# levs57/halo2-liam-eagen-msm

Hardware: AMD Instinct MI355X
Metric: BN254 G1 MSM scalar-point-pairs/s (higher is better)
Workload: dtype u32 limbs (256-bit Montgomery integers)

## Files before the change

halo2_liam_eagen_msm_amd/csrc/kernels.cuh:

```cuda
#pragma once
#include "kernels_ec.cuh"
#include "inv29.cuh"

namespace lemsm {

__device__ __forceinline__ u32 extract_bits(const u32 (&s)[8], u32 bitpos, u32 c) {
  u32 li = bitpos >> 5, sh = bitpos & 31;
  u32 lo = 0, hi = 0;
#pragma unroll
  for (int i = 0; i < 8; i++) {
    lo = ((u32)i == li) ? s[i] : lo;
    hi = ((u32)i == li + 1) ? s[i] : hi;
  }
  u64 v = ((u64)hi << 32) | lo;
  return (u32)(v >> sh) & ((1u << c) - 1u);
}

struct KAdd { u32 k[8]; u32 order[8]; };

template <int MODE ,
          int BS = 256 >
__global__ __launch_bounds__(BS) void k_pip_digits(const uint4* __restrict__ scalars, KAdd kadd, GroupPlan pl,
                                                    uint16_t* __restrict__ dig16, unsigned long long* __restrict__ signbm,
                                                    u32* __restrict__ block_counts,
                                                    u32* __restrict__ bin_total, u32* __restrict__ err) {
  __shared__ u32 hist[MAX_BINS];
  const u32 tid = threadIdx.x, r = blockIdx.x;
  for (u32 i = tid; i < pl.nbins; i += BS) hist[i] = 0;
  __syncthreads();
  const u32 half = 1u << (pl.c - 1);
  u32 j0 = r * pl.spb, j1 = min(j0 + pl.spb, pl.n);
  for (u32 jb = j0 + tid; jb < j1; jb += BS * 4) {
    uint4 a[4], b[4];
#pragma unroll
    for (int u = 0; u < 4; u++) {
      u32 j = jb + (u32)BS * u;
      if (j < j1) { a[u] = scalars[2 * (size_t)j]; b[u] = scalars[2 * (size_t)j + 1]; }
      else { a[u] = make_uint4(0, 0, 0, 0); b[u] = a[u]; }
    }
#pragma unroll
    for (int u = 0; u < 4; u++) {
      u32 j = jb + (u32)BS * u;
      if (j >= j1) continue;
      u32 s[8] = {a[u].x, a[u].y, a[u].z, a[u].w, b[u].x, b[u].y, b[u].z, b[u].w};
      u32 bw = 0;
#pragma unroll
      for (int i = 0; i < 8; i++) { u32 dmy = __builtin_subc(s[i], kadd.order[i], bw, &bw); (void)dmy; }
      if (!bw) {
        atomicAdd(&err[0], 1u); atomicMax(&err[1], ~j);
#pragma unroll
        for (int i = 0; i < 8; i++) s[i] = 0;
      }
      u32 cy = 0;
#pragma unroll
      for (int i = 0; i < 8; i++) s[i] = __builtin_addc(s[i], kadd.k[i], cy, &cy);
      if (MODE == 2) {
#pragma unroll
        for (int w = 0; w < 15; w++) {
          if ((u32)w < pl.w0 || (u32)w >= pl.w1) continue;
          u32 raw = extract_bits(s, 17u * w, 17u);
          u32 sign = ((u32)w + 1 < pl.W && raw < 65536u) ? 1u : 0u;
          u32 mag = ((u32)w + 1 < pl.W) ? (sign ? 65536u - raw : raw - 65536u) : raw;
          dig16[(size_t)((u32)w - pl.w0) * pl.dstride + j] = (uint16_t)(sign ? mag - 1u : mag);
          unsigned long long bal = __ballot(sign != 0);
          if ((threadIdx.x & 63u) == 0) signbm[(size_t)((u32)w - pl.w0) * ((pl.n + 63) / 64) + (j >> 6)] = bal;
          if (mag) atomicAdd(&hist[((u32)w - pl.w0) * pl.BW + ((mag - 1u) >> pl.LB)], 1u);
        }
      } else if (MODE == 1) {
#pragma unroll
        for (int w = 0; w < 16; w++) {
          if ((u32)w < pl.w0 || (u32)w >= pl.w1) continue;
          u32 raw = (w & 1) ? (s[w >> 1] >> 16) : (s[w >> 1] & 0xffffu);
          dig16[(size_t)((u32)w - pl.w0) * pl.dstride + j] = (uint16_t)raw;
          u32 bucket = ((u32)w + 1 < pl.W) ? (raw < half ? half - raw : raw - half) : raw;
          if (bucket) atomicAdd(&hist[((u32)w - pl.w0) * pl.BW + ((bucket - 1u) >> pl.LB)], 1u);
        }
      } else {
        for (u32 w = pl.w0; w < pl.w1; w++) {
          u32 raw = extract_bits(s, w * pl.c, pl.c);
          dig16[(size_t)(w - pl.w0) * pl.dstride + j] = (uint16_t)raw;
          u32 bucket = (w + 1 < pl.W) ? (raw < half ? half - raw : raw - half) : raw;
          if (bucket) atomicAdd(&hist[(w - pl.w0) * pl.BW + ((bucket - 1u) >> pl.LB)], 1u);
        }
      }
    }
  }
  __syncthreads();
  for (u32 i = tid; i < pl.nbins; i += BS) {
    u32 cnt = hist[i];
    u32 wl = i / pl.BW, bin = i - wl * pl.BW;
    const size_t slot = ((size_t)wl * pl.nblk1 + r) * pl.BW + bin;
    block_counts[slot] = cnt;
    block_counts[(size_t)pl.nblk1 * pl.nbins + slot] = cnt ? atomicAdd(&bin_total[i], cnt) : 0u;
  }
}

struct PipDec {
  static constexpr bool VEC = true;
  const uint16_t* dig16;
  const unsigned long long* signbm;
  __device__ __forceinline__ void get(u32 j, u32 w, const GroupPlan& pl, u32& bucket, u32& sign) const {
    u32 raw = dig16[(size_t)(w - pl.w0) * pl.dstride + j];
    if (signbm) {
      sign = (u32)(signbm[(size_t)(w - pl.w0) * ((pl.n + 63) / 64) + (j >> 6)] >> (j & 63u)) & 1u;
      bucket = sign ? raw + 1u : raw;
      return;
    }
    const u32 half = 1u << (pl.c - 1);
    if (w + 1 < pl.W) {
      sign = raw < half ? 1u : 0u;
      bucket = sign ? half - raw : raw - half;
    } else { sign = 0; bucket = raw; }
  }
};
struct NegDec {
  static constexpr bool VEC = false;
  const uint8_t* digitsT;
  __device__ __forceinline__ void get(u32 j, u32 w, const GroupPlan& pl, u32& bucket, u32& sign) const {
    bucket = digitsT[(size_t)w * pl.nstride + j]; sign = 0;
  }
};

__device__ __forceinline__ u32 block_excl_scan_256(u32 v, u32* total, u32* wsum ) {
  const u32 lane = threadIdx.x & 63, wave = threadIdx.x >> 6;
  u32 x = v;
#pragma unroll
  for (int o = 1; o < 64; o <<= 1) {
    u32 y = __shfl_up(x, o);
    if (lane >= (u32)o) x += y;
  }
  if (lane == 63) wsum[wave] = x;
  __syncthreads();
  u32 base = 0, tot = 0;
#pragma unroll
  for (u32 w = 0; w < 4; w++) {
    u32 s = wsum[w];
    if (w < wave) base += s;
    tot += s;
  }
  __syncthreads();
  *total = tot;
  return base + x - v;
}

static const u32 BW_MAX = 512;
static const u32 STAGE = 4096;
static const u32 STAGE2 = 8192;

template <class Dec>
__global__ __launch_bounds__(256) void k_count1(Dec dec, GroupPlan pl, u32* __restrict__ block_counts,
                                                u32* __restrict__ bin_total) {
  __shared__ u32 hist[256];
  const u32 tid = threadIdx.x, wl = blockIdx.x, r = blockIdx.y, w = pl.w0 + wl;
  hist[tid] = 0;
  __syncthreads();
  u32 j0 = r * pl.spb, j1 = min(j0 + pl.spb, pl.n);
  constexpr int PER = STAGE / 256;
  u32 bk[PER];
#pragma unroll
  for (int k = 0; k < PER; k++) {
    u32 j = j0 + tid + 256u * k, sign;
    bk[k] = 0;
    if (j < j1) dec.get(j, w, pl, bk[k], sign);
  }
  const bool few = pl.BW <= 16u;
  const u32 rep = few ? (tid & 15u) << 4 : 0u;
#pragma unroll
  for (int k = 0; k < PER; k++)
    if (bk[k]) atomicAdd(&hist[rep + ((bk[k] - 1u) >> pl.LB)], 1u);
  __syncthreads();
  if (few) {
    u32 c = 0;
    if (tid < 16u) {
#pragma unroll
      for (int r = 0; r < 16; r++) c += hist[r * 16 + tid];
    }
    __syncthreads();
    if (tid < 16u) hist[tid] = c;
    __syncthreads();
  }
  if (tid < pl.BW) {
    u32 cnt = hist[tid];
    const size_t slot = ((size_t)wl * pl.nblk1 + r) * pl.BW + tid;
    block_counts[slot] = cnt;
    block_counts[(size_t)pl.nblk1 * pl.nbins + slot] = cnt ? atomicAdd(&bin_total[wl * pl.BW + tid], cnt) : 0u;
  }
}

__device__ __forceinline__ u32 block_excl_scan_1024(u32 v, u32* total, u32* wsum ) {
  const u32 lane = threadIdx.x & 63, wave = threadIdx.x >> 6;
  u32 x = v;
#pragma unroll
  for (int o = 1; o < 64; o <<= 1) {
    u32 y = __shfl_up(x, o);
    if (lane >= (u32)o) x += y;
  }
  if (lane == 63) wsum[wave] = x;
  __syncthreads();
  u32 base = 0, tot = 0;
  for (u32 w = 0; w < 16; w++) {
    u32 s = wsum[w];
    if (w < wave) base += s;
    tot += s;
  }
  __syncthreads();
  *total = tot;
  return base + x - v;
}

__global__ __launch_bounds__(1024) void k_binscan(GroupPlan pl, const u32* __restrict__ bin_total,
                                                  u32* __restrict__ bin_start, u32* __restrict__ tile_prefix,
                                                  u32* __restrict__ meta) {
  __shared__ u32 wsum[16];
  const u32 t = threadIdx.x;
  constexpr int PB = MAX_BINS / 1024;
  u32 cnt[PB], tl[PB], s = 0, st = 0;
#pragma unroll
  for (int k = 0; k < PB; k++) {
    u32 b = t * PB + k;
    cnt[k] = b < pl.nbins ? bin_total[b] : 0;
    tl[k] = (pl.bin_cap && cnt[k] <= pl.bin_cap) ? 0u : (cnt[k] + pl.T2 - 1) / pl.T2;
    s += cnt[k]; st += tl[k];
  }
  u32 tot, tott;
  u32 off = block_excl_scan_1024(s, &tot, wsum);
  u32 offt = block_excl_scan_1024(st, &tott, wsum);
#pragma unroll
  for (int k = 0; k < PB; k++) {
    u32 b = t * PB + k;
    if (b < pl.nbins) { bin_start[b] = off; tile_prefix[b] = offt; }
    off += cnt[k]; offt += tl[k];
  }
  if (t == 0) {
    bin_start[pl.nbins] = tot; tile_prefix[pl.nbins] = tott;
    meta[META_M] = tot; meta[META_TILES] = tott;
  }
}

template <class Dec, int STG , int BS = 256,
          bool LEAN = false >
__global__ __launch_bounds__(BS) void k_scatter1(Dec dec, GroupPlan pl, const u32* __restrict__ block_counts,
                                                 const u32* __restrict__ bin_start,
                                                 u32* __restrict__ entries, u32 xcd_windows ) {
  static_assert(BS == 256 || BS == 1024, "block size");
  static_assert(STG <= 16384, "jl field is 14 bits");
  static_assert(!LEAN || BS == 256, "the lean form is the 256-thread one");
  __shared__ __align__(8) u32 delta[BW_MAX];
  __shared__ __align__(8) u32 lcur[BW_MAX];
  __shared__ u32 wsum[16];
  __shared__ u32 stage[STG];
  const u32 tid = threadIdx.x;
  u32 wl, r;
  if (xcd_windows) {
    const u32 wpx = (pl.w1 - pl.w0 + 7u) >> 3, slot = blockIdx.x >> 3;
    wl = (blockIdx.x & 7u) + 8u * (slot % wpx); r = slot / wpx;
    if (wl >= pl.w1 - pl.w0) return;
  } else { wl = blockIdx.x; r = blockIdx.y; }
  const u32 w = pl.w0 + wl;
  const u32 lmask = (1u << pl.LB) - 1u;
  u32 j0 = r * pl.spb, j1 = min(j0 + pl.spb, pl.n);
  constexpr int PER = STG / BS;
  u32 bk[PER];
  u32 jl0, jls;
  if constexpr (Dec::VEC) {
    static_assert(PER == 16 || PER == 32, "digits per thread");
    jl0 = tid * PER; jls = 1;
    const u32 jb = j0 + jl0;
    uint4 dv[PER / 8];
    u32 sbits = 0;
    if (jb < j1) {
      const uint4* p = (const uint4*)(dec.dig16 + (size_t)wl * pl.dstride + jb);
#pragma unroll
      for (int v = 0; v < PER / 8; v++) dv[v] = p[v];
      if (dec.signbm) {
        const unsigned long long* sw = dec.signbm + (size_t)wl * ((pl.n + 63) / 64);
        if (PER == 16) sbits = ((const uint16_t*)sw)[jb >> 4]; else sbits = ((const u32*)sw)[jb >> 5];
      }
    } else {
#pragma unroll
      for (int v = 0; v < PER / 8; v++) dv[v] = make_uint4(0, 0, 0, 0);
    }
    const u32 half = 1u << (pl.c - 1);
    const bool top = !(w + 1 < pl.W);
#pragma unroll
    for (int k = 0; k < PER; k++) {
      const uint4 q4 = dv[k / 8];
      const u32 word = ((k / 2) % 4 == 0) ? q4.x : ((k / 2) % 4 == 1) ? q4.y : ((k / 2) % 4 == 2) ? q4.z : q4.w;
      const u32 raw = (k & 1) ? (word >> 16) : (word & 0xffffu);
      u32 bucket, sign;
      if (dec.signbm) { sign = (sbits >> k) & 1u; bucket = raw + sign; }
      else if (top) { sign = 0; bucket = raw; }
      else { sign = raw < half ? 1u : 0u; bucket = sign ? half - raw : raw - half; }
      bk[k] = (jb + (u32)k < j1 && bucket) ? (bucket | (sign << 31)) : 0u;
    }
  } else {
    jl0 = tid; jls = BS;
#pragma unroll
    for (int k = 0; k < PER; k++) {
      u32 j = j0 + tid + (u32)BS * k, b = 0, sgn = 0;
      if (j < j1) dec.get(j, w, pl, b, sgn);
      bk[k] = b ? (b | (sgn << 31)) : 0u;
    }
  }
  const size_t crow = ((size_t)wl * pl.nblk1 + r) * pl.BW;
  const u32* __restrict__ block_offs = block_counts + (size_t)pl.nblk1 * pl.nbins;
  u32 total;
  const bool few = !Dec::VEC && BS == 256 && !LEAN && pl.BW <= 16u;
  if (few) {
    lcur[tid] = 0;
    __syncthreads();
#pragma unroll
    for (int k = 0; k < PER; k++)
      if (bk[k]) atomicAdd(&lcur[((((bk[k] & 0x7fffffffu) - 1u) >> pl.LB) << 4) | (tid & 15u)], 1u);
    __syncthreads();
    const u32 v = lcur[tid];
    const u32 off = block_excl_scan_256(v, &total, wsum);
    lcur[tid] = off;
    const u32 b = tid >> 4;
    if ((tid & 15u) == 0 && b < pl.BW) delta[b] = bin_start[wl * pl.BW + b] + block_offs[crow + b] - off;
  } else
  if constexpr (LEAN) {
    const u32 b0 = 2u * tid;
    const bool h = b0 < pl.BW;
    const uint2 z2 = make_uint2(0u, 0u);
    const uint2 cnt = h ? *reinterpret_cast<const uint2*>(block_counts + crow + b0) : z2;
    const uint2 clm = h ? *reinterpret_cast<const uint2*>(block_offs + crow + b0) : z2;
    const uint2 bs = h ? *reinterpret_cast<const uint2*>(bin_start + (size_t)wl * pl.BW + b0) : z2;
    const u32 off0 = block_excl_scan_256(cnt.x + cnt.y, &total, wsum), off1 = off0 + cnt.x;
    *reinterpret_cast<uint2*>(&delta[b0]) = make_uint2(bs.x + clm.x - off0, bs.y + clm.y - off1);
    *reinterpret_cast<uint2*>(&lcur[b0]) = make_uint2(off0, off1);
  } else if constexpr (BS == 256) {
    const bool h0 = tid < pl.BW, h1 = tid + 256u < pl.BW;
    u32 cnt0 = h0 ? block_counts[crow + tid] : 0u, cnt1 = h1 ? block_counts[crow + tid + 256u] : 0u;
    u32 g0 = h0 ? bin_start[wl * pl.BW + tid] + block_offs[crow + tid] : 0u;
    u32 g1 = h1 ? bin_start[wl * pl.BW + tid + 256u] + block_offs[crow + tid + 256u] : 0u;
    u32 total0, total1;
    u32 off0 = block_excl_scan_256(cnt0, &total0, wsum);
    u32 off1 = block_excl_scan_256(cnt1, &total1, wsum) + total0;
    total = total0 + total1;
    delta[tid] = g0 - off0; delta[tid + 256u] = g1 - off1;
    lcur[tid] = off0; lcur[tid + 256u] = off1;
  } else {
    const bool h0 = tid < pl.BW;
    u32 cnt0 = h0 ? block_counts[crow + tid] : 0u;
    u32 g0 = h0 ? bin_start[wl * pl.BW + tid] + block_offs[crow + tid] : 0u;
    u32 off0 = block_excl_scan_1024(cnt0, &total, wsum);
    if (tid < BW_MAX) { delta[tid] = g0 - off0; lcur[tid] = off0; }
  }
  __syncthreads();
#pragma unroll
  for (int k = 0; k < PER; k++) {
    if (bk[k]) {
      u32 kk = (bk[k] & 0x7fffffffu) - 1u, b = kk >> pl.LB;
      u32 q = atomicAdd(&lcur[few ? ((b << 4) | (tid & 15u)) : b], 1u);
      if constexpr (LEAN) stage[q] = (bk[k] & 0x80000000u) | (jl0 + jls * (u32)k) | (b << 14) | ((kk & lmask) << 24);
      else stage[q] = (jl0 + jls * (u32)k) | ((kk & lmask) << 14) | ((bk[k] >> 31) << 21) | (b << 22);
    }
  }
  __syncthreads();
  if constexpr (LEAN) {
    u32 v[PER];
#pragma unroll
    for (int k = 0; k < PER; k++) { const u32 q = tid + (u32)BS * k; v[k] = q < total ? stage[q] : 0u; }
#pragma unroll
    for (int k = 0; k < PER; k++) {
      const u32 q = tid + (u32)BS * k;
      if (q < total) entries[delta[(v[k] >> 14) & 511u] + q] = (v[k] & 0xff003fffu) + j0;
    }
  } else {
    for (u32 q = tid; q < total; q += BS) {
      u32 v = stage[q];
      entries[delta[v >> 22] + q] = (j0 + (v & 0x3fffu)) | (((v >> 14) & 127u) << 24) | (((v >> 21) & 1u) << 31);
    }
  }
}

__global__ __launch_bounds__(256) void k_tilemap(GroupPlan pl, const u32* __restrict__ bin_start,
                                                 const u32* __restrict__ tile_prefix, const u32* __restrict__ meta,
                                                 uint4* __restrict__ tile_info) {
  u32 t = blockIdx.x * 256 + threadIdx.x;
  if (t >= pl.max_tiles) return;
  if (t >= meta[META_TILES]) { tile_info[t] = make_uint4(0, 0, 0, 0); return; }
  u32 lo = 0, hi = pl.nbins;
  while (hi - lo > 1) {
    u32 mid = (lo + hi) >> 1;
    if (tile_prefix[mid] <= t) lo = mid; else hi = mid;
  }
  u32 off = bin_start[lo] + (t - tile_prefix[lo]) * pl.T2;
  u32 end = min(off + pl.T2, bin_start[lo + 1]);
  tile_info[t] = make_uint4(lo, off, end, 1u);
}
__device__ __forceinline__ bool locate_tile(const uint4* __restrict__ tile_info, u32 t, u32& bin, u32& off, u32& end) {
  uint4 ti = tile_info[t];
  bin = ti.x; off = ti.y; end = ti.z;
  return ti.w != 0;
}

__global__ __launch_bounds__(256) void k_count2(GroupPlan pl, const u32* __restrict__ entries,
                                                const uint4* __restrict__ tile_info, u32* __restrict__ bucket_count) {
  __shared__ u32 hist[1u << MAX_LB];
  const u32 tid = threadIdx.x;
  for (u32 t = blockIdx.x; t < pl.max_tiles; t += gridDim.x) {
    u32 bin, off, end;
    if (!locate_tile(tile_info, t, bin, off, end)) return;
    if (tid < (1u << MAX_LB)) hist[tid] = 0;
    __syncthreads();
    constexpr int PER = STAGE2 / 256;
    u32 e[PER];
#pragma unroll
    for (int k = 0; k < PER; k++) { u32 i = off + tid + 256u * k; e[k] = i < end ? entries[i] : 0xffffffffu; }
#pragma unroll
    for (int k = 0; k < PER; k++) { u32 i = off + tid + 256u * k; if (i < end) atomicAdd(&hist[(e[k] >> 24) & 127u], 1u); }
    __syncthreads();
    if (tid < (1u << pl.LB)) {
      u32 cnt = hist[tid];
      if (cnt) atomicAdd(&bucket_count[(bin << pl.LB) + tid], cnt);
    }
    __syncthreads();
  }
}

__global__ __launch_bounds__(256) void k_bucketscan(GroupPlan pl, const u32* __restrict__ bin_start,
                                                    const u32* __restrict__ bucket_count,
                                                    u32* __restrict__ bucket_start) {
  __shared__ u32 ex[256];
  __shared__ u32 wsum[4];
  const u32 tid = threadIdx.x;
  const u32 key = blockIdx.x * 256 + tid;
  const u32 nkeys = pl.nbins << pl.LB;
  u32 cnt = key < nkeys ? bucket_count[key] : 0u;
  u32 total;
  u32 e = block_excl_scan_256(cnt, &total, wsum);
  ex[tid] = e;
  __syncthreads();
  if (key < nkeys) {
    u32 first = tid & ~((1u << pl.LB) - 1u);
    const u32 b0 = bin_start[key >> pl.LB];
    if (!(pl.bin_cap && bin_start[(key >> pl.LB) + 1] - b0 <= pl.bin_cap))
      bucket_start[key] = b0 + (e - ex[first]);
  }
  if (key == 0) bucket_start[nkeys] = bin_start[pl.nbins];
}

__global__ __launch_bounds__(256) void k_scatter2(GroupPlan pl, const u32* __restrict__ entries,
                                                  const uint4* __restrict__ tile_info, const u32* __restrict__ bucket_start,
                                                  u32* __restrict__ bucket_cursor, u32* __restrict__ sorted) {
  __shared__ u32 hist[256];
  __shared__ u32 lstart[257];
  __shared__ u32 delta[256];
  __shared__ u32 wsum[4];
  __shared__ u32 stage[STAGE2];
  const u32 tid = threadIdx.x;
  for (u32 t = blockIdx.x; t < pl.max_tiles; t += gridDim.x) {
    u32 bin, off, end;
    if (!locate_tile(tile_info, t, bin, off, end)) return;
    hist[tid] = 0;
    __syncthreads();
    constexpr int PER = STAGE2 / 256;
    u32 e[PER], rk[PER];
#pragma unroll
    for (int k = 0; k < PER; k++) { u32 i = off + tid + 256u * k; e[k] = i < end ? entries[i] : 0xffffffffu; }
#pragma unroll
    for (int k = 0; k < PER; k++) {
      u32 i = off + tid + 256u * k;
      rk[k] = i < end ? atomicAdd(&hist[(e[k] >> 24) & 127u], 1u) : 0u;
    }
    __syncthreads();
    u32 cnt = tid < (1u << pl.LB) ? hist[tid] : 0u;
    u32 total;
    u32 o = block_excl_scan_256(cnt, &total, wsum);
    lstart[tid] = o;
    if (tid == 255) lstart[256] = total;
    u32 key = (bin << pl.LB) + tid;
    delta[tid] = cnt ? bucket_start[key] + atomicAdd(&bucket_cursor[key], cnt) - o : 0u;
    __syncthreads();
#pragma unroll
    for (int k = 0; k < PER; k++) {
      u32 i = off + tid + 256u * k;
      if (i < end) {
        u32 l = (e[k] >> 24) & 127u;
        stage[lstart[l] + rk[k]] = e[k];
      }
    }
    __syncthreads();
    for (u32 q = tid; q < total; q += 256) {
      u32 v = stage[q];
      sorted[delta[(v >> 24) & 127u] + q] = v & 0x80ffffffu;
    }
    __syncthreads();
  }
}

static const u32 BIN_CAP = 36864;
static const u32 BIN_CAP_SMALL = 8192;
template <u32 CAP>
__global__ __launch_bounds__(1024) void k_binsort(GroupPlan pl, const u32* __restrict__ entries, const u32* __restrict__ bin_start,
                                                  u32* __restrict__ sorted, u32* __restrict__ bucket_start) {
  __shared__ u32 stage[CAP];
  __shared__ u32 hist[256];
  __shared__ u32 lstart[256];
  __shared__ u32 wsum[4];
  const u32 tid = threadIdx.x, bin = blockIdx.x;
  const u32 off = bin_start[bin], end = bin_start[bin + 1], cnt = end - off;
  if (cnt > pl.bin_cap) return;
  const u32 nl = 1u << pl.LB, lmask = nl - 1u;
  if (tid < 256) hist[tid] = 0;
  __syncthreads();
  constexpr int PER = CAP / 1024;
  u32 e[PER], rk[PER];
#pragma unroll
  for (int k = 0; k < PER; k++) { u32 i = off + tid + 1024u * k; e[k] = i < end ? entries[i] : 0u; }
#pragma unroll
  for (int k = 0; k < PER; k++) {
    u32 i = off + tid + 1024u * k;
    rk[k] = i < end ? atomicAdd(&hist[(e[k] >> 24) & lmask], 1u) : 0u;
  }
  __syncthreads();
  if (tid < 256) {
    u32 c = tid < nl ? hist[tid] : 0u, total;
    const u32 lane = tid & 63, wave = tid >> 6;
    u32 x = c;
#pragma unroll
    for (int o = 1; o < 64; o <<= 1) { u32 y = __shfl_up(x, o); if (lane >= (u32)o) x += y; }
    if (lane == 63) wsum[wave] = x;
    lstart[tid] = x - c;
    (void)total;
  }
  __syncthreads();
  const u32 wb1 = wsum[0], wb2 = wb1 + wsum[1], wb3 = wb2 + wsum[2];
  if (tid < nl) {
    u32 l = tid, base = l < 64 ? 0u : (l < 128 ? wb1 : (l < 192 ? wb2 : wb3));
    bucket_start[(bin << pl.LB) + l] = off + base + lstart[l];
  }
#pragma unroll
  for (int k = 0; k < PER; k++) {
    u32 i = off + tid + 1024u * k;
    if (i < end) {
      u32 l = (e[k] >> 24) & lmask, base = l < 64 ? 0u : (l < 128 ? wb1 : (l < 192 ? wb2 : wb3));
      stage[base + lstart[l] + rk[k]] = e[k] & 0x80ffffffu;
    }
  }
  __syncthreads();
  for (u32 q = tid; q < cnt; q += 1024) sorted[off + q] = stage[q];
}

__global__ void k_copy_points(const CopyTask* __restrict__ tasks, u32 ntasks, u32 nwin, u32 pt_bytes, char* __restrict__ arena) {
  u32 gid = blockIdx.x * blockDim.x + threadIdx.x;
  u32 wpp = pt_bytes / 16;
  u32 word = gid % wpp; u32 r = gid / wpp;
  u32 ti = r / nwin, w = r - ti * nwin;
  if (ti >= ntasks) return;
  CopyTask tk = tasks[ti];
  uint4 v = make_uint4(0, 0, 0, 0);
  if (tk.src_idx < tk.src_valid_idx)
    v = reinterpret_cast<const uint4*>(arena + ((size_t)tk.src_off + (size_t)w * tk.src_wstride + tk.src_idx) * pt_bytes)[word];
  reinterpret_cast<uint4*>(arena + ((size_t)tk.dst_off + (size_t)w * tk.dst_wstride) * pt_bytes)[word] = v;
}

__global__ __launch_bounds__(256) void k_negbase_digits(const uint4* __restrict__ scalars, u32 n, u32 base, u32 d,
                                                        const u32* __restrict__ bound , int check_range,
                                                        uint8_t* __restrict__ digits, uint8_t* __restrict__ digitsT,
                                                        u32* __restrict__ err, u32 row_begin, u32 row_end ,
                                                        const uint8_t* __restrict__ negative = nullptr ,
                                                        uint8_t* __restrict__ trunc = nullptr ) {
  u32 j = blockIdx.x * 256 + threadIdx.x;
  if (j >= n) return;
  uint4 a = scalars[2 * (size_t)j], b = scalars[2 * (size_t)j + 1];
  u32 s[8] = {a.x, a.y, a.z, a.w, b.x, b.y, b.z, b.w};
  u32 bw = 0;
#pragma unroll
  for (int i = 0; i < 8; i++) { u32 dummy = __builtin_subc(s[i], bound[i], bw, &bw); (void)dummy; }
  bool in_range = bw != 0;
  if (check_range && !in_range) { atomicMin(&err[0], j); }
  u32 h[16];
#pragma unroll
  for (int i = 0; i < 8; i++) { h[2 * i] = s[i] & 0xffffu; h[2 * i + 1] = s[i] >> 16; }
  bool neg = negative ? negative[j] != 0 : false;
  {
    u32 nz0 = 0;
#pragma unroll
    for (int k = 0; k < 16; k++) nz0 |= h[k];
    if (!nz0) neg = false;
  }
  const float rb = 1.0f / (float)base;
  const u32 shift = (base & (base - 1u)) == 0 ? (u32)__builtin_ctz(base) : 0u;
  u32 i_begin = 0;
  if (shift && !(s[4] | s[5] | s[6] | s[7])) {
    u32 m0 = s[0], m1 = s[1], m2 = s[2], m3 = s[3];
    for (u32 i = 0; i < d; i++) {
      const u32 rem = m0 & (base - 1u);
      m0 = __builtin_amdgcn_alignbit(m1, m0, shift); m1 = __builtin_amdgcn_alignbit(m2, m1, shift);
      m2 = __builtin_amdgcn_alignbit(m3, m2, shift); m3 >>= shift;
      u32 digit;
      if (!neg) { digit = rem; neg = true; }
      else {
        digit = rem ? base - rem : 0u;
        if (rem) {
          m0 += 1u; const u32 c0 = m0 == 0u; m1 += c0; const u32 c1 = c0 & (m1 == 0u); m2 += c1; const u32 c2 = c1 & (m2 == 0u); m3 += c2;
        }
        neg = false;
      }
      if (!(m0 | m1 | m2 | m3)) neg = false;
      if (digits) digits[(size_t)j * d + i] = (uint8_t)digit;
      if (digitsT && i >= row_begin && i < row_end) digitsT[(size_t)i * n + j] = (uint8_t)digit;
    }
    h[0] = m0 & 0xffffu; h[1] = m0 >> 16; h[2] = m1 & 0xffffu; h[3] = m1 >> 16; h[4] = m2 & 0xffffu; h[5] = m2 >> 16; h[6] = m3 & 0xffffu; h[7] = m3 >> 16;
    i_begin = d;
  }
  for (u32 i = i_begin; i < d; i++) {
    u32 rem = 0;
    if (shift) {
      rem = h[0] & (base - 1u);
#pragma unroll
      for (int k = 0; k < 16; k++) {
        u32 nxt = k < 15 ? h[k + 1] : 0u;
        h[k] = ((h[k] | (nxt << 16)) >> shift) & 0xffffu;
      }
    } else {
#pragma unroll
      for (int k = 15; k >= 0; k--) {
        u32 cur = (rem << 16) | h[k];
        u32 q = (u32)((float)cur * rb);
        int r = (int)cur - (int)(q * base);
        if (r < 0) { q--; r += (int)base; }
        if (r >= (int)base) { q++; r -= (int)base; }
        h[k] = q; rem = (u32)r;
      }
    }
    u32 digit;
    if (!neg) { digit = rem; neg = true; }
    else {
      digit = rem ? base - rem : 0u;
      if (rem) {
        u32 cy = 1;
#pragma unroll
        for (int k = 0; k < 16; k++) { u32 v = h[k] + cy; h[k] = v & 0xffffu; cy = v >> 16; }
      }
      neg = false;
    }
    u32 nz = 0;
#pragma unroll
    for (int k = 0; k < 16; k++) nz |= h[k];
    if (!nz) neg = false;
    if (digits) digits[(size_t)j * d + i] = (uint8_t)digit;
    if (digitsT && i >= row_begin && i < row_end) digitsT[(size_t)i * n + j] = (uint8_t)digit;
  }
  u32 nz = 0;
#pragma unroll
  for (int k = 0; k < 16; k++) nz |= h[k];
  if (nz) { atomicAdd(&err[1], 1u); atomicMin(&err[2], j); }
  if (trunc) trunc[j] = nz ? 1 : 0;
}

struct WitnessPow { unsigned long long lo; long long hi; u32 ovf; u32 pad; };

__device__ __forceinline__ bool add_i128(unsigned long long& lo, long long& hi, unsigned long long blo, long long bhi) {
  unsigned long long rlo = lo + blo;
  long long rhi = (long long)((unsigned long long)hi + (unsigned long long)bhi + (rlo < lo ? 1ull : 0ull));
  bool ovf = ((hi ^ rhi) & (bhi ^ rhi)) < 0;
  lo = rlo; hi = rhi;
  return ovf;
}

__global__ __launch_bounds__(256) void k_scalar_witness(const uint4* __restrict__ scalars, const uint8_t* __restrict__ negative,
                                                        const uint8_t* __restrict__ digits ,
                                                        const uint8_t* __restrict__ trunc, u32 n, u32 base, u32 d, u32 logtable,
                                                        u32 num_limbs, const WitnessPow* __restrict__ powtab,
                                                        char* __restrict__ out, unsigned long long* __restrict__ fail) {
  const u32 j = blockIdx.x * 256 + threadIdx.x;
  if (j >= n) return;
  const u32 cols = num_limbs + 1;
  char* cells = out + (size_t)j * base * cols * 24;
  auto cell = [&](u32 r, u32 c) -> char* { return cells + ((size_t)r * cols + c) * 24; };
  for (u32 r = 0; r < base; r++)
    for (u32 c = 0; c < cols; c++) {
      u32* w = reinterpret_cast<u32*>(cell(r, c));
      w[0] = w[1] = w[2] = w[3] = w[4] = 0;
      w[5] = (c == 0) ? (r == 0 ? 0u : 1u) : 2u;
    }
  auto report = [&](u32 code) { atomicMin(fail, ((unsigned long long)j << 4) | code); };
  if (trunc[j]) { report(1); return; }
  auto add_value = [&](char* c, const WitnessPow& pw) -> bool {
    unsigned long long* v = reinterpret_cast<unsigned long long*>(c);
    unsigned long long lo = v[0]; long long hi = (long long)v[1];
    if (pw.ovf) return true;
    bool o = add_i128(lo, hi, pw.lo, pw.hi);
    v[0] = lo; v[1] = (unsigned long long)hi;
    return o;
  };
  auto add_mask = [&](char* c, u32 k) -> bool {
    if (k >= 32) return true;
    u32* m = reinterpret_cast<u32*>(c + 16);
    u32 a = *m, r = a + (1u << k);
    *m = r;
    return r < a;
  };
  for (u32 i = 0; i < d; i++) {
    u32 dig = digits[(size_t)j * d + i];
    if (!dig) continue;
    const u32 id = dig - 1, k = i % logtable;
    if (add_value(cell(id + 1, 0), powtab[i])) { report(3); return; }
    if (powtab[k].ovf) { report(3); return; }
    if (k + 1 > num_limbs) { report(2); return; }
    if (add_value(cell(id + 1, k + 1), powtab[k])) { report(3); return; }
    if (add_mask(cell(id + 1, k + 1), k)) { report(3); return; }
    if (add_value(cell(0, k + 1), powtab[k])) { report(3); return; }
    if (add_mask(cell(0, k + 1), k)) { report(3); return; }
  }
  {
    uint4 a = scalars[2 * (size_t)j];
    unsigned long long lo = ((unsigned long long)a.y << 32) | a.x, hi = ((unsigned long long)a.w << 32) | a.z;
    if (negative && negative[j]) { lo = ~lo + 1ull; hi = ~hi + (lo == 0 ? 1ull : 0ull); }
    unsigned long long* v = reinterpret_cast<unsigned long long*>(cell(0, 0));
    v[0] = lo; v[1] = hi;
  }
}

template <class F>
__global__ __launch_bounds__(256) void k_table_entries(u32 base, unsigned long long id0, u32 count, uint4* __restrict__ out) {
  const u32 t = blockIdx.x * 256 + threadIdx.x;
  if (t >= count) return;
  typedef typename F::fe fe;
  unsigned long long id = id0 + t;
  fe acc, one, b, bm;
  F::set_zero(acc); F::set_one(one);
  F::set_zero(bm);
  for (int bit = 7; bit >= 0; bit--) { F::add(bm, bm, bm); if ((base >> bit) & 1u) F::add(bm, bm, one); }
  F::neg(b, bm);
  int l = 64 - (id ? __clzll((long long)id) : 64);
  for (int i = l - 1; i >= 0; i--) {
    if ((id >> i) & 1ull) F::add(acc, acc, one);
    F::mul(acc, acc, b);
  }
  F::store(out + 2 * (size_t)t, acc);
}

template <class F, int KB>
__global__ __launch_bounds__(256) void k_jac_to_affine(const uint4* __restrict__ jac, u32 n,
                                                       uint4* __restrict__ aff, char* __restrict__ scratch) {
  typedef typename F::fe fe;
  const u32 t = blockIdx.x * 256 + threadIdx.x;
  const u32 nthreads = gridDim.x * 256;
  const u64 j0 = (u64)t * KB;
  if (j0 >= n) return;
  const u32 cnt = (u32)min((u64)KB, (u64)n - j0);
  fe acc; F::set_one(acc);
  for (u32 k = 0; k < cnt; k++) {
    fe z; F::load(z, jac + (j0 + k) * 6 + 4);
    F::store(scratch + ((size_t)k * nthreads + t) * 32, acc);
    if (!F::is_zero(z)) F::mul(acc, acc, z);
  }
  fe inv; inv_via_lazy<F>(inv, acc);
  for (u32 k = cnt; k-- > 0;) {
    fe x, y, z, pref;
    const uint4* p = jac + (j0 + k) * 6;
    F::load(z, p + 4);
    uint4* o = aff + (j0 + k) * 4;
    if (F::is_zero(z)) {
      o[0] = make_uint4(0, 0, 0, 0); o[1] = o[0]; o[2] = o[0]; o[3] = o[0];
      continue;
    }
    F::load(x, p); F::load(y, p + 2);
    F::load(pref, scratch + ((size_t)k * nthreads + t) * 32);
    fe zi, zi2, zi3;
    F::mul(zi, inv, pref);
    F::mul(inv, inv, z);
    F::sqr(zi2, zi); F::mul(zi3, zi2, zi);
    F::mul(x, x, zi2); F::mul(y, y, zi3);
    F::store(o, x); F::store(o + 2, y);
  }
}

template <class F>
__global__ void k_dbg_montmul(const uint4* __restrict__ a, const uint4* __restrict__ b, uint4* __restrict__ out, u32 n) {
  u32 i = blockIdx.x * blockDim.x + threadIdx.x;
  if (i >= n) return;
  typename F::fe x, y, r;
  F::load(x, a + 2 * (size_t)i); F::load(y, b + 2 * (size_t)i);
  F::mul(r, x, y);
  F::store(out + 2 * (size_t)i, r);
}
template <class F>
__global__ void k_dbg_fieldop(int op, const uint4* __restrict__ a, const uint4* __restrict__ b, uint4* __restrict__ out, u32 n) {
  u32 i = blockIdx.x * blockDim.x + threadIdx.x;
  if (i >= n) return;
  typename F::fe x, y, r;
  F::load(x, a + 2 * (size_t)i); F::load(y, b + 2 * (size_t)i);
  if (op == 0) F::add(r, x, y);
  else if (op == 1) F::sub(r, x, y);
  else if (op == 2) F::neg(r, x);
  else if (op == 3) F::inv(r, x);
  else F::sqr(r, x);
  F::store(out + 2 * (size_t)i, r);
}
template <class F>
__global__ void k_dbg_pointop(int op, const char* __restrict__ acc_in, const char* __restrict__ q_in, char* __restrict__ out, u32 n) {
  typedef XYZZ<F> G;
  u32 i = blockIdx.x * blockDim.x + threadIdx.x;
  if (i >= n) return;
  typename G::pt acc; G::load(acc, acc_in + (size_t)i * 128);
  if (op == 0) {
    typename F::fe x, y; F::load(x, q_in + (size_t)i * 64); F::load(y, q_in + (size_t)i * 64 + 32);
    if (!(F::is_zero(x) && F::is_zero(y))) G::madd(acc, x, y);
  } else {
    typename G::pt q; G::load(q, q_in + (size_t)i * 128);
    G::add(acc, q);
  }
  G::store(out + (size_t)i * 128, acc);
}

}
```

halo2_liam_eagen_msm_amd/csrc/lemsm.hip:

```cpp
#include <hip/hip_runtime.h>
#include <math.h>
#include <stdio.h>
#include <stdlib.h>
#include <string.h>

#include <algorithm>
#include <cmath>
#include <map>
#include <string>
#include <vector>

#include "../../include/lemsm.h"
#include "hostmath.hpp"
#include "hostpool.hpp"
#include "hosttail.hpp"
#include <memory>
#include "kernels.cuh"
#include "rccl_dyn.hpp"
#include "roctx_dyn.hpp"
#include "divisor.cuh"
#include <rocprim/rocprim.hpp>
#include <chrono>
#include <functional>
#include <thread>

using namespace lemsm;

namespace {

typedef Field32<FqParams> FqDev;
typedef Field32<FrParams> FrDev;
typedef XYZZ<FqDev> GqStrict;
typedef XYZZ<FrDev> GrStrict;
typedef XYZZ29<Field29<Fq29Params>> GqLazy;
typedef XYZZ29<Field29<Fr29Params>> GrLazy;

const u32 ORDER_R[8] = {0xf0000001u, 0x43e1f593u, 0x79b97091u, 0x2833e848u, 0x8181585du, 0xb85045b6u, 0xe131a029u, 0x30644e72u};
const u32 ORDER_P[8] = {0xd87cfd47u, 0x3c208c16u, 0x6871ca8du, 0x97816a91u, 0x8181585du, 0xb85045b6u, 0xe131a029u, 0x30644e72u};
const u32 BOUND_R[8] = {0xc7b81b1bu, 0xc6fb4e9fu, 0xeeb859fcu, 0x6f4d8248u, 0, 0, 0, 0};
const u32 BOUND_P[8] = {0xc7b81b1cu, 0xc6fb4e9fu, 0xeeb859fcu, 0x6f4d8248u, 0, 0, 0, 0};

const u32* order_of(int curve) { return curve == LEMSM_BN254_G1 ? ORDER_R : ORDER_P; }
const u32* bound_of(int curve) { return curve == LEMSM_BN254_G1 ? BOUND_R : BOUND_P; }

}
#define LEMSM_EXTERN_G(G)                                                                                   \
  extern template __global__ void lemsm::k_merge_pairs<G>(GroupPlan, u32, MqLayout, const u32*, const u32*, const u32*, const char*, char*, u32*, uint4*); \
  extern template __global__ void lemsm::k_merge_serial<G>(u32, MqLayout, const u32*, const uint4*, const char*, char*); \
  extern template __global__ void lemsm::k_merge_waves<G>(u32, MqLayout, const u32*, const uint4*, const char*, char*, char*, u32*); \
  extern template __global__ void lemsm::k_merge_final<G>(u32, MqLayout, const u32*, const uint4*, const char*, char*, u32*); \
  extern template __global__ void lemsm::k_pyramid<G>(const PyrTask*, u32, u32, u32, char*, u32); \
  extern template __global__ void lemsm::k_pyramid_first2<G>(PyrFirst2Args, const u32*, char*, u32*); \
  extern template __global__ void lemsm::k_pyramid_tail<G>(const PyrTask*, PyrTailArgs, const CopyTaskPod*, u32, char*, u32);
#define LEMSM_EXTERN_ACC(G, W) \
  extern template __global__ void lemsm::k_accum1<G, W>(GroupPlan, const u32*, const u32*, u32*, const uint4*, char*, u32*, char*);
LEMSM_EXTERN_G(GqStrict) LEMSM_EXTERN_G(GrStrict) LEMSM_EXTERN_G(GqLazy) LEMSM_EXTERN_G(GrLazy)
LEMSM_EXTERN_ACC(GqStrict, 4) LEMSM_EXTERN_ACC(GrStrict, 4)
LEMSM_EXTERN_ACC(GqLazy, 2) LEMSM_EXTERN_ACC(GqLazy, 3) LEMSM_EXTERN_ACC(GqLazy, 4)
LEMSM_EXTERN_ACC(GrLazy, 2) LEMSM_EXTERN_ACC(GrLazy, 3) LEMSM_EXTERN_ACC(GrLazy, 4)
extern template __global__ void lemsm::k_accum1<GqLazy, 3, true>(GroupPlan, const u32*, const u32*, u32*, const uint4*, char*, u32*, char*);
extern template __global__ void lemsm::k_accum1<GrLazy, 3, true>(GroupPlan, const u32*, const u32*, u32*, const uint4*, char*, u32*, char*);
extern template __global__ void lemsm::k_accum1<GqLazy, 3, true, true>(GroupPlan, const u32*, const u32*, u32*, const uint4*, char*, u32*, char*);
extern template __global__ void lemsm::k_accum1<GrLazy, 3, true, true>(GroupPlan, const u32*, const u32*, u32*, const uint4*, char*, u32*, char*);
extern template __global__ void lemsm::k_convert_points<Field29<Fq29Params>>(const uint4*, uint4*, u32);
extern template __global__ void lemsm::k_convert_points<Field29<Fr29Params>>(const uint4*, uint4*, u32);
namespace {

struct DevBuf {
  void* p = nullptr;
  size_t cap = 0;
};


struct PyrCacheEntry { DevBuf buf; PyrPlan pp; };

}

struct HostStage { const uint8_t* h_scalars; const void* h_points; char* d_scalars; char* d_points; };

struct lemsm_ctx {
  int device = 0;
  u32 num_cus = 256;
  hipStream_t stream = nullptr;
  hipStream_t stream_sort = nullptr;
  hipStream_t stream_tail = nullptr;
  std::vector<hipEvent_t> evpool;
  hipEvent_t wait_accum = nullptr;
  hipEvent_t ev_call_done = nullptr;
  hipEvent_t ev_batch_up = nullptr;
  hipEvent_t dw_ev[2] = {nullptr, nullptr};
  hipEvent_t ev[5] = {nullptr, nullptr, nullptr, nullptr, nullptr};
  DevBuf ws;
  DevBuf in_s;
  DevBuf in_p;
  DevBuf in_aux;
  DevBuf gather;
  DevBuf fail_buf;
  DevBuf dw_tab, dw_arena, dw_tmp;
  u32 dw_logn = 0, dw_gexp = 0;
  double dw_ntt_ms = 0; u64 dw_ntt_bytes = 0, dw_ntt_bflies = 0; u32 dw_reuse_levels = 0;
  double dw_phase_ms[4] = {0, 0, 0, 0};
  ncclComm_t comm = nullptr; int comm_size = 1, comm_rank = 0;
  int plan_world = 1;
  u32* h_small = nullptr;
  lemsm_ctx* peer = nullptr;
  void* h_pin = nullptr; size_t h_pin_cap = 0;
  std::unique_ptr<lemsm::host::Pool> pool;
  std::string last_error;
  long opt_host_threads = 0;
  long opt_window_bits = 0, opt_chunk = 0, opt_tile = 0, opt_field = 0, opt_accum_waves = 0, opt_groups = 0, opt_host_slab_bits = 0, opt_slab_bits = 0, opt_abi_points = 0, opt_stage2x = 0, opt_xcd_windows = 0, opt_entry_ring = 0, opt_validate_points = 0, opt_pyr_fuse = 0, opt_ntt_tiled = 0, opt_ws_canary = 0, opt_binsort = 0, opt_dw_wrap = 0, opt_dw_fuse = 0, opt_dw_kb = 0, opt_merge_slice = 0, opt_merge_wave_th = 0, opt_dbg_repeat = 0, opt_pyr_first2 = 0, opt_dw_reuse = 0, opt_dw_pw_lazy = 0, opt_dw_halves = 0, opt_dw_ntt_lazy = 0, opt_slab_tail = 0, opt_pyr_quad = 0, opt_scatter_lean = 0;
  u32 plan_slab_n = 0;
  bool plan_ring = false;
  const struct HostStage* host_stage = nullptr;
  double t_total_ms = 0, t_accum_ms = 0; int n_accum = 0;
  double host_us[4] = {0, 0, 0, 0};
  uint32_t dbg_stamps[8] = {0, 0, 0, 0, 0, 0, 0, 0};
  uint64_t dbg_merge[4] = {0, 0, 0, 0};
  double accum_clock_mhz = 0;
  size_t bad_index = 0;
  size_t truncated = 0;
  std::map<std::vector<u32>, PyrCacheEntry> pyr_cache;
};

namespace {

#define HIPCHK(ctx, expr)                                                                   \
  do {                                                                                      \
    hipError_t e_ = (expr);                                                                 \
    if (e_ != hipSuccess) {                                                                 \
      (ctx)->last_error = std::string(#expr) + ": " + hipGetErrorString(e_);                \
      return LEMSM_ERR_HIP;                                                                 \
    }                                                                                       \
  } while (0)

int fail(lemsm_ctx* ctx, int code, const std::string& msg) {
  if (ctx) ctx->last_error = msg;
  return code;
}

int reserve(lemsm_ctx* ctx, DevBuf& b, size_t bytes) {
  if (b.cap >= bytes) return LEMSM_OK;
  if (b.p) { HIPCHK(ctx, hipFree(b.p)); b.p = nullptr; b.cap = 0; }
  size_t want = bytes + bytes / 8 + 4096;
  hipError_t e = hipMalloc(&b.p, want);
  if (e != hipSuccess) { b.p = nullptr; return fail(ctx, LEMSM_ERR_NOMEM, "hipMalloc failed: " + std::string(hipGetErrorString(e))); }
  b.cap = want;
  return LEMSM_OK;
}

int reserve_pinned(lemsm_ctx* ctx, size_t bytes) {
  if (ctx->h_pin_cap >= bytes) return LEMSM_OK;
  if (ctx->h_pin) { HIPCHK(ctx, hipHostFree(ctx->h_pin)); ctx->h_pin = nullptr; ctx->h_pin_cap = 0; }
  size_t want = bytes + bytes / 4 + 4096;
  hipError_t e = hipHostMalloc(&ctx->h_pin, want, hipHostMallocDefault);
  if (e != hipSuccess) { ctx->h_pin = nullptr; return fail(ctx, LEMSM_ERR_NOMEM, "hipHostMalloc failed: " + std::string(hipGetErrorString(e))); }
  ctx->h_pin_cap = want;
  return LEMSM_OK;
}

void host_parallel(lemsm_ctx* ctx, int njobs, const std::function<void(int)>& fn) {
  if (!ctx || njobs <= 1 || ctx->opt_host_threads == 1) { for (int i = 0; i < njobs; i++) fn(i); return; }
  int want = ctx->opt_host_threads > 1 ? (int)ctx->opt_host_threads : std::min(8, lemsm::host::Pool::usable_cpus());
  if (!ctx->pool || ctx->pool->workers() != want - 1) ctx->pool.reset(new lemsm::host::Pool(std::max(0, want - 1)));
  ctx->pool->run(njobs, fn);
}

bool geq8(const u32* a, const u32* b) {
  for (int i = 7; i >= 0; i--) { if (a[i] > b[i]) return true; if (a[i] < b[i]) return false; }
  return true;
}
void add8(u32* r, const u32* a, const u32* b) {
  u64 c = 0;
  for (int i = 0; i < 8; i++) { c += (u64)a[i] + b[i]; r[i] = (u32)c; c >>= 32; }
}
u32 logb_ceil8(const u32* x, u32 base) {
  u32 m[8]; memcpy(m, x, 32); u32 i = 0;
  for (;;) {
    u32 nz = 0; for (int k = 0; k < 8; k++) nz |= m[k];
    if (!nz) break;
    u64 rem = 0;
    for (int k = 7; k >= 0; k--) { u64 cur = (rem << 32) | m[k]; m[k] = (u32)(cur / base); rem = cur % base; }
    i++;
  }
  return i;
}
u32 next_pow2(u32 x) { u32 p = 1; while (p < x) p <<= 1; return p; }
u32 ilog2(u32 x) { u32 l = 0; while ((1u << l) < x) l++; return l; }

struct MsmPlan {
  u32 c, W, nb, nbp, L;
  u32 kadd[8];
};

u32 choose_c(const lemsm_ctx* ctx, size_t n) {
  if (ctx && ctx->opt_window_bits >= 2 && ctx->opt_window_bits <= 17) return (u32)ctx->opt_window_bits;
  u32 lg = 0; while (((size_t)1 << (lg + 1)) <= n) lg++;
  if (lg >= 24) return (ctx && ctx->plan_world > 1) ? 16u : 17u;
  int c = (int)lg - 3;
  if (c < 3) c = 3;
  if (c > 16) c = 16;
  return (u32)c;
}

u32 host_slab_log(const lemsm_ctx* ctx, size_t n) {
  u32 lg = 0; while (((size_t)2 << lg) <= n) lg++;
  u32 auto_log = std::min(21u, std::max(19u, lg >= 2 ? lg - 2 : 0u));
  if (ctx->host_stage && !ctx->host_stage->h_points) auto_log = std::min(22u, std::max(19u, lg >= 2 ? lg - 2 : 0u));
  return std::min<u32>(MAX_SLAB_LOG, ctx->opt_host_slab_bits ? (u32)ctx->opt_host_slab_bits : auto_log);
}

MsmPlan make_msm_plan(const lemsm_ctx* ctx, int curve, size_t n) {
  MsmPlan p; memset(&p, 0, sizeof p);
  size_t n_pass = n;
  if (ctx && ctx->host_stage) n_pass = std::min(n, (size_t)1 << host_slab_log(ctx, n));
  else if (ctx && ctx->opt_slab_bits) n_pass = std::min(n, (size_t)1 << ctx->opt_slab_bits);
  p.c = choose_c(ctx, n_pass);
  p.nb = 1u << (p.c - 1);
  p.nbp = p.nb; p.L = ilog2(p.nbp);
  const u32* order = order_of(curve);
  for (u32 W = (254 + p.c - 1) / p.c;; W++) {
    u32 K[8] = {0, 0, 0, 0, 0, 0, 0, 0};
    for (u32 w = 0; w + 1 < W; w++) {
      u32 bit = w * p.c + p.c - 1;
      if (bit < 256) K[bit >> 5] |= 1u << (bit & 31);
    }
    u32 s[9]; u64 cy = 0;
    for (int i = 0; i < 8; i++) { cy += (u64)order[i] + K[i]; s[i] = (u32)cy; cy >>= 32; }
    s[8] = (u32)cy;
    u32 sh = p.c * (W - 1);
    bool fits = true;
    if (s[8]) fits = false;
    u64 top = 0; bool big = false;
    for (int bit = 255; bit >= (int)sh; bit--) {
      u32 b = (s[bit >> 5] >> (bit & 31)) & 1u;
      if (top >> 62) big = true;
      top = (top << 1) | b;
    }
    if (big || top > p.nb) fits = false;
    if (sh >= 256) { fits = true; }
    if (fits) { p.W = W; memcpy(p.kadd, K, 32); break; }
  }
  if (p.c == 17 && p.W != 15) {
    lemsm_ctx tmp_opts; tmp_opts.opt_window_bits = 16;
    return make_msm_plan(&tmp_opts, curve, n);
  }
  return p;
}

template <class F> struct FieldTag {};

size_t align_up(size_t x, size_t a) { return (x + a - 1) / a * a; }

struct GroupWs {
  u32* err;
  char* arena;
  u32* bin_total; u32* bin_cursor; u32* bin_start; u32* tile_prefix; u32* meta;
  u32* bucket_count; u32* bucket_cursor; u32* bucket_start;
  u32* block_counts;
  uint16_t* dig16;
  unsigned long long* signbm;
  uint4* tile_info;
  u32* entries; u32* sorted;
  u32* rec_key; char* rec_pt;
  u32* mq_cnt; uint4* mq_items; char* mq_partial; MqLayout mq;
  size_t zero_begin, zero_bytes;
  size_t zero_bytes_counters;
  size_t total;
  std::vector<size_t> guards;
};

MqLayout make_mq_layout(const lemsm_ctx* ctx, u32 nthr1) {
  return make_mq_layout_t(nthr1, ctx && ctx->opt_merge_slice ? (u32)ctx->opt_merge_slice : 512u,
                          ctx && ctx->opt_merge_wave_th ? (u32)ctx->opt_merge_wave_th - 1u : 2048u);
}

const size_t WS_GUARD = 256;
GroupWs carve(char* base, const GroupPlan& pl, const ArenaLayout& ar, const MqLayout& mq, size_t ptb, bool guard = false) {
  GroupWs w; size_t off = 0;
  auto take = [&](size_t bytes) {
    size_t o = off;
    if (guard) { size_t g = align_up(off + bytes, 16); w.guards.push_back(g); off = align_up(g + WS_GUARD, 256); }
    else off = align_up(off + bytes, 256);
    return o;
  };
  u32 NBpad = pl.nbins << pl.LB;
  size_t z0 = off;
  size_t o_err = take(64);
  size_t o_mqcnt = take(MQ_WORDS * 4);
  size_t o_bin_total = take(MAX_BINS * 4), o_bin_cursor = take(MAX_BINS * 4);
  size_t o_bcount = take((size_t)NBpad * 4), o_bcursor = take((size_t)NBpad * 4);
  size_t o_arena = take((size_t)ar.total_points * ptb);
  size_t zend = o_arena + (size_t)(ar.apyr_off - ar.bucket_off) * ptb;
  w.zero_bytes_counters = o_arena - z0;
  size_t o_bin_start = take((MAX_BINS + 1) * 4), o_tile_prefix = take((MAX_BINS + 1) * 4), o_meta = take(64);
  size_t o_bstart = take(((size_t)NBpad + 1) * 4);
  size_t o_blockc = take((size_t)pl.nblk1 * pl.nbins * 8);
  size_t o_dig = take(pl.c ? (size_t)pl.dstride * (pl.w1 - pl.w0) * 2 + 64 : 16);
  size_t o_tinfo = take((size_t)pl.max_tiles * 16 + 16);
  size_t o_sbm = take(pl.c == 17 ? (size_t)(pl.w1 - pl.w0) * ((pl.n + 63) / 64) * 8 + 16 : 16);
  size_t Mmax = (size_t)pl.n * (pl.w1 - pl.w0);
  size_t o_entries = take(Mmax * 4 + 4 * (size_t)pl.L1 + 512), o_sorted = take(Mmax * 4 + 4 * (size_t)pl.L1 + 512);
  w.mq = mq;
  size_t o_rk = take((size_t)pl.nthr1 * 4 + 16), o_rp = take(2 * (size_t)pl.nthr1 * ptb + 256);
  size_t o_mqi = take(((size_t)mq.offF + mq.capF) * 16), o_mqp = take((size_t)mq.capP * ptb + 256);
  w.total = off;
  if (base) {
    w.err = (u32*)(base + o_err);
    w.bin_total = (u32*)(base + o_bin_total); w.bin_cursor = (u32*)(base + o_bin_cursor);
    w.bucket_count = (u32*)(base + o_bcount); w.bucket_cursor = (u32*)(base + o_bcursor);
    w.arena = base + o_arena;
    w.bin_start = (u32*)(base + o_bin_start); w.tile_prefix = (u32*)(base + o_tile_prefix); w.meta = (u32*)(base + o_meta);
    w.bucket_start = (u32*)(base + o_bstart); w.block_counts = (u32*)(base + o_blockc); w.dig16 = (uint16_t*)(base + o_dig); w.tile_info = (uint4*)(base + o_tinfo); w.signbm = (unsigned long long*)(base + o_sbm);
    w.entries = (u32*)(base + o_entries); w.sorted = (u32*)(base + o_sorted);
    w.rec_key = (u32*)(base + o_rk); w.rec_pt = base + o_rp;
    w.mq_cnt = (u32*)(base + o_mqcnt); w.mq_items = (uint4*)(base + o_mqi); w.mq_partial = base + o_mqp;
  }
  w.zero_begin = z0; w.zero_bytes = zend - z0;
  return w;
}

u32 choose_lb(const lemsm_ctx* ctx, u32 nb, u32 n, u32 d) {
  if (ctx && ctx->plan_slab_n) n = ctx->plan_slab_n;
  u32 LB = 0;
  while (((nb + (1u << LB) - 1) >> LB) > 256 && LB < MAX_LB) LB++;
  if (d == 0 && ctx && ctx->opt_binsort != 2 && LB > 0) {
    const u32 cap = ctx->opt_binsort > 2 ? std::min((u32)ctx->opt_binsort, (u32)BIN_CAP) : (u32)BIN_CAP;
    const u32 BW = (nb + (1u << LB) - 1) >> LB;
    if ((u64)n / BW > (u64)cap * 9 / 10 && 2 * BW <= BW_MAX && (u64)n / (2 * BW) <= (u64)cap * 9 / 10) LB--;
  }
  return LB;
}

GroupPlan make_group_plan(const lemsm_ctx* ctx, u32 n, u32 c, u32 nb, u32 W, u32 w0, u32 w1, u32 d) {
  GroupPlan g; memset(&g, 0, sizeof g);
  g.n = n; g.c = c; g.nb = nb; g.W = W; g.w0 = w0; g.w1 = w1; g.d = d; g.nstride = n;
  u32 LB = choose_lb(ctx, nb, n, d);
  g.LB = LB;
  g.BW = (nb + (1u << LB) - 1) >> LB;
  g.nbw = g.BW << LB;
  g.NB = (w1 - w0) * g.nbw;
  g.nbins = (w1 - w0) * g.BW;
  u32 spb = (n + 1023) / 1024;
  spb = std::max(256u, std::min((u32)STAGE, spb));
  spb = (spb + 255) / 256 * 256;
  if (n >= (1u << 16)) spb = STAGE;
  if (n >= (1u << 16) && d == 0 && ctx->opt_stage2x == 4) spb = 4 * STAGE;
  if (n >= (1u << 16) && d == 0 && ctx->opt_stage2x == 2) spb = 2 * STAGE;
  g.spb = spb;
  g.dstride = (n + 63u) / 64u * 64u;
  g.nblk1 = (n + spb - 1) / spb;
  if (g.nblk1 == 0) g.nblk1 = 1;
  size_t Mmax = (size_t)n * (w1 - w0);
  u32 T2 = ctx->opt_tile > 0 ? std::min((u32)ctx->opt_tile, (u32)STAGE2) : (u32)STAGE2;
  g.T2 = T2;
  g.max_tiles = (u32)(Mmax / T2) + g.nbins + 1;
  g.bin_cap = ctx->opt_binsort == 2 ? 0u : (ctx->opt_binsort > 2 ? std::min((u32)ctx->opt_binsort, (u32)BIN_CAP) : (u32)BIN_CAP);
  if (g.bin_cap == BIN_CAP && g.BW && (u64)n * 3 / 2 / g.BW <= BIN_CAP_SMALL) g.bin_cap = BIN_CAP_SMALL;
  u32 L1;
  if (ctx->opt_chunk > 0) L1 = (u32)ctx->opt_chunk;
  else {
    size_t target = (size_t)256 * 4 * 3 * 64 * 2;
    size_t l = (Mmax + target - 1) / target;
    L1 = (u32)std::max((size_t)8, std::min((size_t)256, l));
  }
  if (ctx->plan_ring && ctx->opt_chunk == 0 && L1 >= 128) L1 = (L1 + 15u) & ~15u;
  g.L1 = L1;
  g.nthr1 = (u32)((Mmax + L1 - 1) / L1);
  if (g.nthr1 == 0) g.nthr1 = 1;
  return g;
}

u32 max_group_windows(const lemsm_ctx* ctx, u32 nb, u32 n, u32 d) {
  u32 LB = choose_lb(ctx, nb, n, d);
  u32 BW = (nb + (1u << LB) - 1) >> LB;
  u32 cap = MAX_BINS / BW;
  return cap == 0 ? 1 : cap;
}

struct PipProvider {
  const uint4* scalars; KAdd kadd;
  typedef PipDec Dec;
  int prepare(lemsm_ctx*, hipStream_t st, const GroupPlan& pl, uint16_t* dig16, unsigned long long* signbm, u32* block_counts,
              u32* bin_total, u32* err, Dec& dec) const {
    dec.dig16 = dig16; dec.signbm = nullptr;
    if (pl.c == 17) {
      dec.signbm = signbm;
      if (pl.nblk1 < 2048)
        hipLaunchKernelGGL((k_pip_digits<2, 1024>), dim3(pl.nblk1), dim3(1024), 0, st, scalars, kadd, pl, dig16, signbm, block_counts, bin_total, err);
      else
        hipLaunchKernelGGL((k_pip_digits<2>), dim3(pl.nblk1), dim3(256), 0, st, scalars, kadd, pl, dig16, signbm, block_counts, bin_total, err);
    } else if (pl.c == 16 && pl.W == 16) {
      if (pl.nblk1 < 1024)
        hipLaunchKernelGGL((k_pip_digits<1, 1024>), dim3(pl.nblk1), dim3(1024), 0, st, scalars, kadd, pl, dig16, signbm, block_counts, bin_total, err);
      else
        hipLaunchKernelGGL((k_pip_digits<1>), dim3(pl.nblk1), dim3(256), 0, st, scalars, kadd, pl, dig16, signbm, block_counts, bin_total, err);
    } else {
      if (pl.nblk1 < 1024)
        hipLaunchKernelGGL((k_pip_digits<0, 1024>), dim3(pl.nblk1), dim3(1024), 0, st, scalars, kadd, pl, dig16, signbm, block_counts, bin_total, err);
      else
        hipLaunchKernelGGL((k_pip_digits<0>), dim3(pl.nblk1), dim3(256), 0, st, scalars, kadd, pl, dig16, signbm, block_counts, bin_total, err);
    }
    return LEMSM_OK;
  }
};
struct NegProvider {
  const uint8_t* digitsT;
  typedef NegDec Dec;
  int prepare(lemsm_ctx*, hipStream_t st, const GroupPlan& pl, uint16_t*, unsigned long long*, u32* block_counts, u32* bin_total, u32*, Dec& dec) const {
    dec.digitsT = digitsT;
    hipLaunchKernelGGL((k_count1<NegDec>), dim3(pl.w1 - pl.w0, pl.nblk1), dim3(256), 0, st, dec, pl, block_counts, bin_total);
    return LEMSM_OK;
  }
};

__global__ __launch_bounds__(256) void k_group_finish(const uint4* __restrict__ out_area, uint4* __restrict__ d_out, u32 n16,
                                                      const u32* __restrict__ err, const u32* __restrict__ clock, const u32* __restrict__ mq_cnt,
                                                      u32* __restrict__ slot) {
  const u32 i = blockIdx.x * 256 + threadIdx.x;
  if (i < n16) d_out[i] = out_area[i];
  if (blockIdx.x == 0 && threadIdx.x < 24) {
    const u32 k = threadIdx.x;
    slot[k] = k < 2 ? err[k] : (k < 4 ? 0u : (k < 12 ? clock[k - 4] : (k < 16 ? mq_cnt[k - 12] : mq_cnt[k - 8])));
  }
}

template <class G, class Prov>
int run_group(lemsm_ctx* ctx, const Prov& prov, const GroupPlan& pl, u32 nbp, u32 L, const void* d_points,
              bool abi ,
              char* ws_base, char* d_out , u32* d_slot , hipStream_t s_sort, hipStream_t s_acc,
              hipStream_t s_tail, hipEvent_t ev_sorted, hipEvent_t ev_acc0, hipEvent_t ev_acc1,
              hipEvent_t ev_points  = nullptr,
              u32 slab_k = 0, u32 nba = 1 , u32 scaled_mask = 0 ) {
  hipStream_t st = s_sort;
  u32 gw = pl.w1 - pl.w0;
  u32 NBpad = pl.nbins << pl.LB;
  ArenaLayout ar = make_arena(NBpad, nbp, gw, L, nba);
  const bool abi_pyr = nba > 1 ? false : abi;
  const bool last_slab = slab_k + 1 == nba;
  std::vector<u32> pkey = {NBpad, pl.nb, pl.nbw, nbp, L, gw, abi_pyr ? 1u : 0u, nba};
  auto pit = ctx->pyr_cache.find(pkey);
  if (pit == ctx->pyr_cache.end()) {
    PyrCacheEntry ent;
    ent.pp = make_pyr_plan(ar, pl.nb, pl.nbw, nbp, L, abi_pyr);
    std::vector<PyrTask> flat;
    for (auto& s : ent.pp.steps) flat.insert(flat.end(), s.begin(), s.end());
    size_t tb = align_up(flat.size() * sizeof(PyrTask), 256);
    int rcr = reserve(ctx, ent.buf, tb + sizeof(CopyTask) + 64); if (rcr) return rcr;
    HIPCHK(ctx, hipMemcpy(ent.buf.p, flat.data(), flat.size() * sizeof(PyrTask), hipMemcpyHostToDevice));
    HIPCHK(ctx, hipMemcpy((char*)ent.buf.p + tb, &ent.pp.copy, sizeof(CopyTask), hipMemcpyHostToDevice));
    pit = ctx->pyr_cache.emplace(pkey, std::move(ent)).first;
  }
  const PyrPlan& pp = pit->second.pp;
  size_t ntasks_total = 0;
  for (auto& s : pp.steps) ntasks_total += s.size();
  PyrTask* d_tasks = (PyrTask*)pit->second.buf.p;
  CopyTask* d_copy = (CopyTask*)((char*)pit->second.buf.p + align_up(ntasks_total * sizeof(PyrTask), 256));
  const size_t ptb = G::PT_BYTES;
  const MqLayout mq = make_mq_layout(ctx, pl.nthr1);
  GroupWs w = carve(ws_base, pl, ar, mq, ptb, ctx->opt_ws_canary != 0);
  if (pl.nbins > MAX_BINS || pl.BW > BW_MAX || pl.LB > MAX_LB || pl.spb > 4 * STAGE || (pl.c && pl.dstride < pl.n) || pl.T2 > STAGE2 || pl.bin_cap > BIN_CAP)
    return fail(ctx, LEMSM_ERR_HIP, "internal: window-group plan exceeds a kernel limit (bins " + std::to_string(pl.nbins) + ", bins per window " + std::to_string(pl.BW) + ")");

  const bool first2 = L >= 5 && ctx->opt_pyr_first2 == 1 && nba == 1;
  RoctxRange rg_group("lemsm: window group (digits + sort + accumulate + tail enqueued)");
  HIPCHK(ctx, hipMemsetAsync(ws_base + w.zero_begin, 0, (first2 || slab_k > 0) ? w.zero_bytes_counters : w.zero_bytes, st));
  for (size_t g : w.guards) HIPCHK(ctx, hipMemsetAsync(ws_base + g, 0xA5, WS_GUARD, st));

  typename Prov::Dec dec;
  { int rcp = prov.prepare(ctx, st, pl, w.dig16, w.signbm, w.block_counts, w.bin_total, w.err, dec); if (rcp) return rcp; }
  hipLaunchKernelGGL(k_binscan, dim3(1), dim3(1024), 0, st, pl, w.bin_total, w.bin_start, w.tile_prefix, w.meta);
  const u32 xw = (gw >= 8 && ctx->opt_xcd_windows != 1) ? 1u : 0u;
  dim3 g1 = xw ? dim3(8u * ((gw + 7) / 8) * pl.nblk1) : dim3(gw, pl.nblk1);
  if (pl.spb > 2 * STAGE)
    hipLaunchKernelGGL((k_scatter1<typename Prov::Dec, 4 * STAGE, 1024>), g1, dim3(1024), 0, st, dec, pl, w.block_counts, w.bin_start, w.entries, xw);
  else if (pl.spb > STAGE)
    hipLaunchKernelGGL((k_scatter1<typename Prov::Dec, 2 * STAGE>), g1, dim3(256), 0, st, dec, pl, w.block_counts, w.bin_start, w.entries, xw);
  else if (Prov::Dec::VEC && (pl.BW & 1u) == 0 && ctx->opt_scatter_lean == 1)
    hipLaunchKernelGGL((k_scatter1<typename Prov::Dec, STAGE, 256, true>), g1, dim3(256), 0, st, dec, pl, w.block_counts, w.bin_start, w.entries, xw);
  else
    hipLaunchKernelGGL((k_scatter1<typename Prov::Dec, STAGE>), g1, dim3(256), 0, st, dec, pl, w.block_counts, w.bin_start, w.entries, xw);
  const u32* d_sorted = w.entries;
  const u32* d_bstart = w.bin_start;
  if (pl.LB > 0) {
    if (pl.bin_cap && pl.bin_cap <= BIN_CAP_SMALL) hipLaunchKernelGGL((k_binsort<BIN_CAP_SMALL>), dim3(pl.nbins), dim3(1024), 0, st, pl, w.entries, w.bin_start, w.sorted, w.bucket_start);
    else if (pl.bin_cap) hipLaunchKernelGGL((k_binsort<BIN_CAP>), dim3(pl.nbins), dim3(1024), 0, st, pl, w.entries, w.bin_start, w.sorted, w.bucket_start);
    hipLaunchKernelGGL(k_tilemap, dim3((pl.max_tiles + 255) / 256), dim3(256), 0, st, pl, w.bin_start, w.tile_prefix, w.meta, w.tile_info);
    const u32 g2 = pl.bin_cap ? std::min(pl.max_tiles, 768u) : pl.max_tiles;
    hipLaunchKernelGGL(k_count2, dim3(g2), dim3(256), 0, st, pl, w.entries, w.tile_info, w.bucket_count);
    hipLaunchKernelGGL(k_bucketscan, dim3(((pl.nbins << pl.LB) + 255) / 256), dim3(256), 0, st, pl, w.bin_start, w.bucket_count, w.bucket_start);
    hipLaunchKernelGGL(k_scatter2, dim3(g2), dim3(256), 0, st, pl, w.entries, w.tile_info,
                       w.bucket_start, w.bucket_cursor, w.sorted);
    d_sorted = w.sorted; d_bstart = w.bucket_start;
  }

  HIPCHK(ctx, hipEventRecord(ev_sorted, s_sort));
  st = s_acc;
  HIPCHK(ctx, hipStreamWaitEvent(s_acc, ev_sorted, 0));
  if (ev_points) HIPCHK(ctx, hipStreamWaitEvent(s_acc, ev_points, 0));
  if (ctx->wait_accum) HIPCHK(ctx, hipStreamWaitEvent(s_acc, ctx->wait_accum, 0));
  HIPCHK(ctx, hipEventRecord(ev_acc0, s_acc));
  {
    dim3 grid((pl.nthr1 + 255) / 256), blk(256);
    char* bsum = w.arena + ((size_t)ar.bucket_off + (size_t)slab_k * NBpad) * ptb;
    int wps = G::CONVERTED_DOMAIN ? (ctx->opt_accum_waves ? (int)ctx->opt_accum_waves : 3) : 4;
    if constexpr (G::CONVERTED_DOMAIN) {
      if (wps == 2) hipLaunchKernelGGL((k_accum1<G, 2>), grid, blk, 0, st, pl, d_sorted, d_bstart, w.meta, (const uint4*)d_points, bsum, w.rec_key, w.rec_pt);
      else if (wps == 4) hipLaunchKernelGGL((k_accum1<G, 4>), grid, blk, 0, st, pl, d_sorted, d_bstart, w.meta, (const uint4*)d_points, bsum, w.rec_key, w.rec_pt);
      else if (abi && (pl.L1 & 15u) == 0 && pl.L1 >= 32 && ctx->opt_entry_ring != 1) hipLaunchKernelGGL((k_accum1<G, 3, true, true>), grid, blk, 0, st, pl, d_sorted, d_bstart, w.meta, (const uint4*)d_points, bsum, w.rec_key, w.rec_pt);
      else if (abi) hipLaunchKernelGGL((k_accum1<G, 3, true>), grid, blk, 0, st, pl, d_sorted, d_bstart, w.meta, (const uint4*)d_points, bsum, w.rec_key, w.rec_pt);
      else hipLaunchKernelGGL((k_accum1<G, 3>), grid, blk, 0, st, pl, d_sorted, d_bstart, w.meta, (const uint4*)d_points, bsum, w.rec_key, w.rec_pt);
    } else {
      hipLaunchKernelGGL((k_accum1<G, 4>), grid, blk, 0, st, pl, d_sorted, d_bstart, w.meta, (const uint4*)d_points, bsum, w.rec_key, w.rec_pt);
    }
  }
  HIPCHK(ctx, hipEventRecord(ev_acc1, s_acc));
  st = s_tail;
  HIPCHK(ctx, hipStreamWaitEvent(s_tail, ev_acc1, 0));

  {
    RoctxRange rg_tail("lemsm: edge-record merge");
    const u32 sc = abi ? 1u : 0u;
    char* bsum = w.arena + ((size_t)ar.bucket_off + (size_t)slab_k * NBpad) * ptb;
    hipLaunchKernelGGL((k_merge_pairs<G>), dim3((pl.nthr1 + 255) / 256), dim3(256), 0, st, pl, sc, mq, d_bstart, w.meta, w.rec_key, w.rec_pt, bsum, w.mq_cnt, w.mq_items);
    hipLaunchKernelGGL((k_merge_serial<G>), dim3(std::min(ctx->num_cus, std::max(1u, (mq.capS + mq.capM + 63) / 64))), dim3(256), 0, st, sc, mq, w.mq_cnt, w.mq_items, w.rec_pt, bsum);
    hipLaunchKernelGGL((k_merge_waves<G>), dim3(std::min(ctx->num_cus, std::max(1u, (mq.capM + mq.capL + 3) / 4))), dim3(256), 0, st, sc, mq, w.mq_cnt, w.mq_items, w.rec_pt, w.mq_partial, bsum, w.mq_cnt);
    hipLaunchKernelGGL((k_merge_final<G>), dim3(std::min(ctx->num_cus, std::max(1u, (mq.capF + 3) / 4))), dim3(256), 0, st, sc, mq, w.mq_cnt, w.mq_items, w.mq_partial, bsum, w.mq_cnt);
  }
  RoctxRange rg_pyr("lemsm: bucket-reduction pyramid");
  if (nba > 1 && last_slab)
    hipLaunchKernelGGL((k_sum_slabs<G>), dim3((NBpad + 255) / 256), dim3(256), 0, st, w.arena + (size_t)ar.bucket_off * ptb, NBpad, nba, scaled_mask);
  if (last_slab) {
    size_t toff = 0;
    u32 s_begin = 1;
    if (first2) {
      PyrFirst2Args fa; memset(&fa, 0, sizeof fa);
      fa.nwin = gw; fa.nb = pl.nb; fa.nbw = pl.nbw; fa.nbp = nbp; fa.bucket_off = ar.bucket_off; fa.wstride = nbp;
      fa.a2_off = ar.apyr_off + nbp / 2;
      fa.r02_off = ar.rbuf_off + nbp / 4;
      fa.r11_off = ar.rbuf_off + nbp / 2;
      fa.scaled = abi_pyr ? 1u : 0u;
      const u32 threads = gw * (nbp / 8);
      hipLaunchKernelGGL((k_pyramid_first2<G>), dim3((threads + 255) / 256), dim3(256), 0, st, fa, d_bstart, w.arena, w.mq_cnt);
      toff = pp.steps[0].size() + pp.steps[1].size();
      s_begin = 3;
    }
    u32 first_fused = L + 1;
    if (ctx->opt_pyr_fuse != 1) {
      const size_t lim = ctx->opt_pyr_fuse == 2 ? 2048 : 256;
      for (u32 s = s_begin; s <= L; s++) {
        bool fits = true;
        for (u32 q = s; q <= L; q++) if ((size_t)pp.steps[q - 1].size() * pp.step_max_count[q - 1] > lim) fits = false;
        if (fits && L - s + 1 <= 20) { first_fused = s; break; }
      }
      if (first_fused == L) first_fused = L + 1;
    }
    for (u32 s = s_begin; s <= L && s < first_fused; s++) {
      auto& tasks = pp.steps[s - 1];
      u32 maxc = pp.step_max_count[s - 1];
      size_t threads = (size_t)tasks.size() * maxc * gw;
      const u32 quad = (G::CONVERTED_DOMAIN && ctx->opt_pyr_quad != 2 && threads <= 32768 && !(s == 1 && abi_pyr)) ? 1u : 0u;
      if (quad) threads *= 4;
      hipLaunchKernelGGL((k_pyramid<G>), dim3((u32)((threads + 255) / 256)), dim3(256), 0, st, d_tasks + toff, (u32)tasks.size(), gw, maxc, w.arena, quad);
      toff += tasks.size();
    }
    const bool need_copy = !(L == 1 && abi_pyr);
    if (first_fused <= L) {
      PyrTailArgs ta; memset(&ta, 0, sizeof ta);
      ta.first = first_fused; ta.last = L;
      u32 o = (u32)toff;
      for (u32 s = first_fused; s <= L; s++) { ta.step_off[s - first_fused] = o; ta.max_count[s - first_fused] = pp.step_max_count[s - 1]; o += (u32)pp.steps[s - 1].size(); }
      ta.step_off[L - first_fused + 1] = o;
      hipLaunchKernelGGL((k_pyramid_tail<G>), dim3(gw), dim3(1024), 0, st, (const PyrTask*)d_tasks, ta, (const CopyTaskPod*)d_copy, need_copy ? 1u : 0u, w.arena,
                         (G::CONVERTED_DOMAIN && ctx->opt_pyr_quad != 2) ? 1u : 0u);
    } else if (need_copy) {
      u32 cthreads = gw * (u32)(ptb / 16);
      hipLaunchKernelGGL(k_copy_points, dim3((cthreads + 63) / 64), dim3(64), 0, st, d_copy, 1u, gw, (u32)ptb, w.arena);
    }
  }
  {
    const u32 n16 = last_slab ? (u32)((size_t)gw * (L + 1) * ptb / 16) : 0u;
    hipLaunchKernelGGL(k_group_finish, dim3(std::max(1u, (n16 + 255) / 256)), dim3(256), 0, st, (const uint4*)(w.arena + (size_t)ar.out_off * ptb), (uint4*)d_out, n16,
                       w.err, w.meta + META_CLOCK, w.mq_cnt, d_slot);
  }
  HIPCHK(ctx, hipGetLastError());
  if (!w.guards.empty()) {
    std::vector<unsigned char> host(w.guards.size() * WS_GUARD);
    for (size_t i = 0; i < w.guards.size(); i++) HIPCHK(ctx, hipMemcpyAsync(host.data() + i * WS_GUARD, ws_base + w.guards[i], WS_GUARD, hipMemcpyDeviceToHost, st));
    HIPCHK(ctx, hipStreamSynchronize(s_sort)); HIPCHK(ctx, hipStreamSynchronize(s_acc)); HIPCHK(ctx, hipStreamSynchronize(st));
    for (size_t i = 0; i < host.size(); i++)
      if (host[i] != 0xA5) return fail(ctx, LEMSM_ERR_HIP, "workspace guard " + std::to_string(i / WS_GUARD) + " overwritten at byte " + std::to_string(i % WS_GUARD) + " (option ws_canary)");
  }
  return LEMSM_OK;
}

size_t group_ws_bytes(const lemsm_ctx* ctx, const GroupPlan& pl, u32 nbp, u32 L, size_t ptb, bool guard, u32 nba = 1) {
  u32 gw = pl.w1 - pl.w0;
  ArenaLayout ar = make_arena(pl.nbins << pl.LB, nbp, gw, L, nba);
  GroupWs w = carve(nullptr, pl, ar, make_mq_layout(ctx, pl.nthr1), ptb, guard);
  return w.total + 4096;
}


struct WinRun {
  size_t nslabs = 0, ng = 0, out_slab = 0, SLAB = 0, err_slot = 0;
  size_t nrec = 0;
  size_t err_stride = 1;
  size_t err_cap = 0;
  char* d_out = nullptr; char* d_err = nullptr;
  u32 nw = 0, nw_pad = 0, L = 0; size_t ptb = 0;
  size_t send_bytes() const { return out_slab * nrec; }
  static constexpr size_t STATUS_BYTES = 256;
  size_t send_total() const { return out_slab * nrec + err_cap + STATUS_BYTES; }
};

bool shared_tail(const lemsm_ctx* ctx, size_t nslabs) { return nslabs > 1 && nslabs <= 8 && ctx->opt_slab_tail != 2 && ctx->opt_groups <= 1; }

template <class G>
void win_sizes(const lemsm_ctx* ctx, size_t n, u32 nw_pad, u32 L, WinRun& wr) {
  const u32 slab_log = ctx->opt_slab_bits ? (u32)ctx->opt_slab_bits : MAX_SLAB_LOG;
  wr.SLAB = (size_t)1 << slab_log;
  wr.nslabs = n ? (n + wr.SLAB - 1) / wr.SLAB : 1;
  wr.nrec = shared_tail(ctx, wr.nslabs) ? 1 : wr.nslabs;
  wr.ptb = G::PT_BYTES; wr.L = L; wr.nw_pad = nw_pad; wr.nw = 0; wr.ng = 0;
  wr.out_slab = align_up((size_t)std::max(nw_pad, 1u) * (L + 1) * wr.ptb, 256);
  wr.err_slot = 96; wr.err_stride = std::max<size_t>(nw_pad, 1);
  wr.err_cap = align_up(wr.nslabs * wr.err_stride * wr.err_slot, 256);
  wr.d_out = nullptr; wr.d_err = nullptr;
}

void comm_abort(lemsm_ctx* ctx) {
  if (!ctx->comm) return;
  Rccl& rc = Rccl::get();
  if (rc.CommAbort) (void)rc.CommAbort(ctx->comm); else (void)rc.CommDestroy(ctx->comm);
  ctx->comm = nullptr; ctx->comm_size = 1; ctx->comm_rank = 0;
  ctx->last_error += " [communicator aborted: this rank could not enter the exchange]";
}

template <class P64, class G, class MakeSrc>
int run_windows_enqueue(lemsm_ctx* ctx, MakeSrc make_src, size_t n, u32 c, u32 nb, u32 nbp, u32 L, u32 W, u32 wb, u32 we, u32 d,
                        const void* d_points, u32 nw_pad, WinRun& wr) {
  u32 nw = we - wb;
  if (nw_pad < nw) nw_pad = nw;
  ctx->plan_ring = false;
  const HostStage* hs = ctx->host_stage;
  u32 slab_log = ctx->opt_slab_bits ? (u32)ctx->opt_slab_bits : MAX_SLAB_LOG;
  if (hs) slab_log = host_slab_log(ctx, n);
  const size_t SLAB = (size_t)1 << slab_log;
  const size_t nslabs = n ? (n + SLAB - 1) / SLAB : 1;
  const bool shared = shared_tail(ctx, nslabs);
  const u32 nba = shared ? (u32)nslabs : 1u;
  const size_t nrec = shared ? 1 : nslabs;
  ctx->plan_slab_n = (u32)std::min(SLAB, n);
  u32 gmax = max_group_windows(ctx, nb, ctx->plan_slab_n, d);
  const size_t ptb = G::PT_BYTES;
  u32 ngroups = 1;
  if (ctx->opt_groups > 0) ngroups = std::min((u32)ctx->opt_groups, std::max(nw, 1u));
  u32 gsz = std::max(1u, std::min(gmax, (nw + ngroups - 1) / ngroups));
  struct Grp { u32 g0, g1; size_t off; };
  std::vector<Grp> groups;
  size_t ws_total = 0;
  if (n) {
    u32 sn0 = (u32)std::min(SLAB, n), snl = (u32)(n - (nslabs - 1) * SLAB);
    for (u32 g0 = wb; g0 < we; g0 += gsz) {
      u32 g1 = std::min(we, g0 + gsz);
      size_t bytes = group_ws_bytes(ctx, make_group_plan(ctx, sn0, c, nb, W, g0, g1, d), nbp, L, ptb, ctx->opt_ws_canary != 0, nba);
      if (snl != sn0) bytes = std::max(bytes, group_ws_bytes(ctx, make_group_plan(ctx, snl, c, nb, W, g0, g1, d), nbp, L, ptb, ctx->opt_ws_canary != 0, nba));
      groups.push_back({g0, g1, ws_total});
      ws_total += align_up(bytes + 8192, 256);
    }
  }
  const size_t ng = groups.size();
  const size_t out_slab = align_up((size_t)std::max(nw_pad, 1u) * (L + 1) * ptb, 256);
  const size_t ERR_SLOT = 96;
  const size_t err_stride = std::max<size_t>(nw_pad, 1);
  const size_t err_bytes = align_up(nslabs * err_stride * ERR_SLOT, 256);
  size_t conv_bytes = G::CONVERTED_DOMAIN ? align_up(std::min(SLAB, n) * 64, 256) : 0;
  wr.nslabs = nslabs; wr.nrec = nrec; wr.ng = ng; wr.out_slab = out_slab; wr.SLAB = SLAB; wr.err_slot = ERR_SLOT; wr.err_stride = err_stride; wr.err_cap = err_bytes;
  wr.nw = nw; wr.nw_pad = nw_pad; wr.L = L; wr.ptb = ptb;
  int rc = reserve(ctx, ctx->ws, ws_total + conv_bytes + out_slab * nrec + err_bytes + WinRun::STATUS_BYTES + 4096);
  if (rc) return rc;
  char* ws_base = (char*)ctx->ws.p;
  char* d_conv = ws_base + ws_total;
  char* d_out = d_conv + conv_bytes;
  char* d_err = d_out + out_slab * nrec;
  wr.d_out = d_out; wr.d_err = d_err;
  while (ctx->evpool.size() < 3 * ng * nslabs + (hs ? nslabs : 0)) {
    hipEvent_t e; HIPCHK(ctx, hipEventCreate(&e)); ctx->evpool.push_back(e);
  }
  hipEvent_t* ev_up = ctx->evpool.data() + 3 * ng * nslabs;
  hipStream_t s_sort = ctx->stream_sort, s_acc = ctx->stream, s_tail = ctx->stream_tail;
  const bool one_queue = ctx->opt_groups <= 1;
  if (one_queue) { s_sort = s_acc; s_tail = s_acc; }
  hipStream_t s_up = ctx->stream_sort;
  if (hs && !one_queue) return fail(ctx, LEMSM_ERR_BAD_ARG, "option groups > 1 is only available on the device-pointer entries");
  if (!one_queue) HIPCHK(ctx, hipStreamSynchronize(s_acc));
  HIPCHK(ctx, hipEventRecord(ctx->ev[0], s_acc));
  ctx->t_accum_ms = 0; ctx->n_accum = 0;
  if (nw_pad != nw || n == 0 || nw == 0)
    HIPCHK(ctx, hipMemsetAsync(d_out, 0, out_slab * nrec, s_acc));
  HIPCHK(ctx, hipMemsetAsync(d_err, 0, err_bytes + WinRun::STATUS_BYTES, s_acc));
  u32 scaled_mask = 0;
  for (size_t k = 0; k < nslabs && n && nw; k++) {
    const size_t s0 = k * SLAB;
    u32 sn = (u32)std::min(SLAB, n - s0);
    if (hs) {
      HIPCHK(ctx, hipMemcpyAsync(hs->d_scalars + s0 * 32, hs->h_scalars + s0 * 32, (size_t)sn * 32, hipMemcpyHostToDevice, s_up));
      if (hs->h_points)
        HIPCHK(ctx, hipMemcpyAsync(hs->d_points + s0 * 64, (const char*)hs->h_points + s0 * 64, (size_t)sn * 64, hipMemcpyHostToDevice, s_up));
      HIPCHK(ctx, hipEventRecord(ev_up[k], s_up));
      HIPCHK(ctx, hipStreamWaitEvent(s_acc, ev_up[k], 0));
    }
    const char* pts = (const char*)d_points + s0 * 64;
    bool abi = false;
    hipEvent_t ev_points = nullptr;
    ctx->plan_ring = false;
    if constexpr (G::CONVERTED_DOMAIN) {
      GroupPlan pl0 = make_group_plan(ctx, sn, c, nb, W, groups[0].g0, groups[0].g1, d);
      double S = std::max(1.0, std::min((double)pl0.L1, (double)sn / (double)nb));
      double P = 1.0 - std::pow(1.0 - 1.0 / S, 64.0);
      abi = P * (double)(groups[0].g1 - groups[0].g0) < 7.0 && (ctx->opt_accum_waves == 0 || ctx->opt_accum_waves == 3);
      if (ctx->opt_abi_points == 1) abi = false;
      if (ctx->opt_abi_points == 2) abi = (ctx->opt_accum_waves == 0 || ctx->opt_accum_waves == 3);
      ctx->plan_ring = abi && ctx->opt_entry_ring != 1;
      if (!abi) {
        if (one_queue && !hs) {
          HIPCHK(ctx, hipEventRecord(ctx->ev[2], s_acc));
          HIPCHK(ctx, hipStreamWaitEvent(ctx->stream_sort, ctx->ev[2], 0));
          hipLaunchKernelGGL((k_convert_points<typename G::F_>), dim3((2 * sn + 255) / 256), dim3(256), 0, ctx->stream_sort, (const uint4*)pts, (uint4*)d_conv, sn);
          HIPCHK(ctx, hipEventRecord(ctx->ev[3], ctx->stream_sort));
          ev_points = ctx->ev[3];
        } else {
          hipLaunchKernelGGL((k_convert_points<typename G::F_>), dim3((2 * sn + 255) / 256), dim3(256), 0, s_acc, (const uint4*)pts, (uint4*)d_conv, sn);
        }
        pts = d_conv;
      }
    }
    for (size_t gi = 0; gi < ng; gi++) {
      const Grp& gr = groups[gi];
      GroupPlan pl = make_group_plan(ctx, sn, c, nb, W, gr.g0, gr.g1, d);
      pl.nstride = (u32)n;
      auto src = make_src(s0, sn);
      hipEvent_t* ev = ctx->evpool.data() + 3 * (k * ng + gi);
      if (gi == 0 && abi) scaled_mask |= 1u << k;
      rc = run_group<G>(ctx, src, pl, nbp, L, pts, abi, ws_base + gr.off, d_out + (shared ? 0 : k) * out_slab + (size_t)(gr.g0 - wb) * (L + 1) * ptb,
                        (u32*)(d_err + (k * err_stride + gi) * ERR_SLOT), s_sort, s_acc, s_tail, ev[0], ev[1], ev[2], gi == 0 ? ev_points : nullptr,
                        shared ? (u32)k : 0u, nba, scaled_mask);
      if (rc) return rc;
    }
    if (!one_queue) {
      HIPCHK(ctx, hipStreamSynchronize(s_sort));
      HIPCHK(ctx, hipStreamSynchronize(s_acc));
      HIPCHK(ctx, hipStreamSynchronize(s_tail));
    }
  }
  if (n == 0 || nw == 0) { wr.ng = 0; }
  return LEMSM_OK;
}

hipStream_t records_stream(const lemsm_ctx* ctx) { return ctx->opt_groups <= 1 ? ctx->stream : ctx->stream_tail; }

int collect_local_stats(lemsm_ctx* ctx, const WinRun& wr, const u32* slots) {
  u64 clk_cyc = 0, clk_ticks = 0;
  const size_t sw = wr.err_slot / 4;
  for (int q = 0; q < 4; q++) ctx->dbg_merge[q] = 0;
  for (size_t k = 0; k < wr.nslabs; k++)
    for (size_t gi = 0; gi < wr.ng; gi++) {
      const u32* ew = slots + (k * wr.err_stride + gi) * sw;
      const size_t i = k * wr.ng + gi;
      for (int q = 0; q < 4; q++) ctx->dbg_merge[q] += ew[12 + q];
      for (int q = 0; q < 8; q++) ctx->dbg_stamps[q] = ew[16 + q];
      float a = 0; HIPCHK(ctx, hipEventElapsedTime(&a, ctx->evpool[3 * i + 1], ctx->evpool[3 * i + 2]));
      ctx->t_accum_ms += a; ctx->n_accum++;
      u64 ck[4]; memcpy(ck, ew + 4, 32);
      if (ck[2] > ck[0] && ck[3] > ck[1] && ck[2] - ck[0] < ((u64)1 << 40)) { clk_cyc += ck[2] - ck[0]; clk_ticks += ck[3] - ck[1]; }
    }
  ctx->accum_clock_mhz = clk_ticks ? (double)clk_cyc / (double)clk_ticks * 100.0 : 0.0;
  return LEMSM_OK;
}

size_t first_bad_scalar(const WinRun& wr, const u32* slots) {
  size_t best = SIZE_MAX;
  const size_t sw = wr.err_slot / 4;
  for (size_t k = 0; k < wr.nslabs; k++)
    for (size_t gi = 0; gi < wr.err_stride; gi++) {
      const u32* ew = slots + (k * wr.err_stride + gi) * sw;
      if (ew[0]) best = std::min(best, k * wr.SLAB + (size_t)(~ew[1]));
    }
  return best;
}

int run_windows_finish(lemsm_ctx* ctx, const WinRun& wr, const char* d_raw, size_t raw_bytes, std::vector<char>& raw) {
  RoctxRange rg_fin("lemsm: read-back and wait");
  hipStream_t s_tail = records_stream(ctx);
  raw.resize(raw_bytes);
// ... 380 lines not shown
  std::vector<host::pt> sums;
  window_sums_par<P64>(ctx, all.data(), lp.d, lp.L, sums);
  lhs_combine_t<P64>(lp, sums.data(), out_carry, out_carries);
  return LEMSM_OK;
}

int msm_sharded_dispatch(lemsm_ctx* ctx, int curve, const void* d_scalars, const void* d_points, size_t n, const Exchange& ex, u64 out[12]) {
  if (n == 0) { memset(out, 0, 96); return LEMSM_OK; }
  int saved = ctx->plan_world; ctx->plan_world = ex.world;
  int rc;
  if (ctx->opt_field == 1) {
    rc = curve == LEMSM_BN254_G1 ? msm_sharded_t<host::FqParams64, GqStrict>(ctx, curve, d_scalars, d_points, n, ex, out)
                                 : msm_sharded_t<host::FrParams64, GrStrict>(ctx, curve, d_scalars, d_points, n, ex, out);
  } else {
    rc = curve == LEMSM_BN254_G1 ? msm_sharded_t<host::FqParams64, GqLazy>(ctx, curve, d_scalars, d_points, n, ex, out)
                                 : msm_sharded_t<host::FrParams64, GrLazy>(ctx, curve, d_scalars, d_points, n, ex, out);
  }
  ctx->plan_world = saved;
  return rc;
}
int lhs_sharded_dispatch(lemsm_ctx* ctx, int curve, const void* d_scalars, const void* d_points, size_t n, const LhsPlan& lp,
                         const Exchange& ex, u64 out_carry[12], u64* out_carries, size_t* bad_index) {
  if (ctx->opt_field == 1) {
    if (curve == LEMSM_BN254_G1) return lhs_sharded_t<host::FqParams64, GqStrict>(ctx, curve, d_scalars, d_points, n, lp, ex, out_carry, out_carries, bad_index);
    return lhs_sharded_t<host::FrParams64, GrStrict>(ctx, curve, d_scalars, d_points, n, lp, ex, out_carry, out_carries, bad_index);
  }
  if (curve == LEMSM_BN254_G1) return lhs_sharded_t<host::FqParams64, GqLazy>(ctx, curve, d_scalars, d_points, n, lp, ex, out_carry, out_carries, bad_index);
  return lhs_sharded_t<host::FrParams64, GrLazy>(ctx, curve, d_scalars, d_points, n, lp, ex, out_carry, out_carries, bad_index);
}

template <class F>
__global__ __launch_bounds__(256) void k_precompute_mult(const uint4* __restrict__ jac, u32 n, u32 base, uint4* __restrict__ out) {
  typedef XYZZ<F> G; typedef typename F::fe fe;
  u32 j = blockIdx.x * 256 + threadIdx.x;
  if (j >= n) return;
  fe X, Y, Z; F::load(X, jac + (size_t)j * 6); F::load(Y, jac + (size_t)j * 6 + 2); F::load(Z, jac + (size_t)j * 6 + 4);
  typename G::pt p;
  if (F::is_zero(Z)) G::set_identity(p);
  else { p.x = X; p.y = Y; F::sqr(p.zz, Z); F::mul(p.zzz, p.zz, Z); }
  typename G::pt acc = p;
  for (u32 k = 1; k < base; k++) {
    uint4* o = out + ((size_t)j * (base - 1) + (k - 1)) * 6;
    if (G::is_identity(acc)) { uint4 z = make_uint4(0, 0, 0, 0); for (int q = 0; q < 6; q++) o[q] = z; }
    else {
      fe t, xo, yo;
      F::sqr(t, acc.zz); F::mul(xo, acc.x, t);
      F::sqr(t, acc.zzz); F::mul(yo, acc.y, t);
      F::store(o, xo); F::store(o + 2, yo); F::store(o + 4, acc.zzz);
    }
    G::add(acc, p);
  }
}

template <class F>
__global__ __launch_bounds__(256) void k_precompute_mult_affine(const uint4* __restrict__ jac, u32 n, u32 base,
                                                                uint4* __restrict__ out, char* __restrict__ scratch) {
  typedef XYZZ<F> G; typedef typename F::fe fe;
  u32 j = blockIdx.x * 256 + threadIdx.x;
  if (j >= n) return;
  fe X, Y, Z; F::load(X, jac + (size_t)j * 6); F::load(Y, jac + (size_t)j * 6 + 2); F::load(Z, jac + (size_t)j * 6 + 4);
  typename G::pt p;
  if (F::is_zero(Z)) G::set_identity(p);
  else { p.x = X; p.y = Y; F::sqr(p.zz, Z); F::mul(p.zzz, p.zz, Z); }
  typename G::pt acc = p;
  fe pref; F::set_one(pref);
  for (u32 k = 1; k < base; k++) {
    char* s = scratch + ((size_t)(k - 1) * n + j) * 160;
    G::store(s, acc); F::store(s + 128, pref);
    if (!G::is_identity(acc)) F::mul(pref, pref, acc.zzz);
    G::add(acc, p);
  }
  fe inv; inv_via_lazy<F>(inv, pref);
  for (u32 k = base - 1; k >= 1; k--) {
    const char* s = scratch + ((size_t)(k - 1) * n + j) * 160;
    typename G::pt q; G::load(q, s); fe pr; F::load(pr, s + 128);
    uint4* o = out + ((size_t)j * (base - 1) + (k - 1)) * 4;
    if (G::is_identity(q)) { uint4 z = make_uint4(0, 0, 0, 0); o[0] = z; o[1] = z; o[2] = z; o[3] = z; continue; }
    fe izzz, izz, x, y;
    F::mul(izzz, inv, pr);
    F::mul(inv, inv, q.zzz);
    F::mul(izz, izzz, q.zz); F::sqr(izz, izz);
    F::mul(x, q.x, izz); F::mul(y, q.y, izzz);
    F::store(o, x); F::store(o + 2, y);
  }
}

template <class F, int KB>
__global__ __launch_bounds__(256) void k_gen_walk(const uint4* __restrict__ q_aff, u32 n, uint4* __restrict__ out, char* __restrict__ scratch) {
  typedef XYZZ<F> G; typedef typename F::fe fe;
  const u32 t = blockIdx.x * 256 + threadIdx.x;
  const u32 nthreads = gridDim.x * 256;
  const u64 j0 = (u64)t * KB;
  if (j0 >= n) return;
  const u32 cnt = (u32)min((u64)KB, (u64)n - j0);
  fe qx, qy; F::load(qx, q_aff); F::load(qy, q_aff + 2);
  typename G::pt acc; G::set_identity(acc);
  u32 k = (u32)j0 + 1;
  for (int b = 31; b >= 0; b--) {
    if (!G::is_identity(acc)) { typename G::pt tmp = acc; G::dbl(acc, tmp); }
    if ((k >> b) & 1u) G::madd(acc, qx, qy);
  }
  fe pref; F::set_one(pref);
  for (u32 i = 0; i < cnt; i++) {
    if (i) G::madd(acc, qx, qy);
    char* s = scratch + ((size_t)i * nthreads + t) * 160;
    G::store(s, acc); F::store(s + 128, pref);
    F::mul(pref, pref, acc.zzz);
  }
  fe inv; inv_via_lazy<F>(inv, pref);
  for (u32 i = cnt; i-- > 0;) {
    const char* s = scratch + ((size_t)i * nthreads + t) * 160;
    typename G::pt p; G::load(p, s); fe pr; F::load(pr, s + 128);
    fe izzz, izz, x, y;
    F::mul(izzz, inv, pr);
    F::mul(inv, inv, p.zzz);
    F::mul(izz, izzz, p.zz); F::sqr(izz, izz);
    F::mul(x, p.x, izz); F::mul(y, p.y, izzz);
    F::store(out + (j0 + i) * 4, x); F::store(out + (j0 + i) * 4 + 2, y);
  }
}

template <class F29>
__device__ __forceinline__ void dbg_in29(typename F29::fe& r, const void* p) { typename F29::fe a; F29::load(a, p); F29::from_abi(r, a); }
template <class F29>
__device__ __forceinline__ void dbg_out29(void* p, const typename F29::fe& a) { typename F29::fe t; F29::div32(t, a); F29::store(p, t); }

template <class F29>
__global__ void k_dbg_fieldop29(int op, const uint4* __restrict__ a, const uint4* __restrict__ b, uint4* __restrict__ out, u32 n) {
  u32 i = blockIdx.x * blockDim.x + threadIdx.x;
  if (i >= n) return;
  typename F29::fe x, y, r;
  dbg_in29<F29>(x, a + 2 * (size_t)i); dbg_in29<F29>(y, b + 2 * (size_t)i);
  if (op == 0) { F29::add(r, x, y); F29::wnorm(r); }
  else if (op == 1) F29::sub(r, x, y);
  else if (op == 2) F29::neg(r, x);
  else if (op == 4) F29::sqr(r, x);
  else if (op == 5) F29::mul2(r, x, y, y, x);
  else if (op == 6) F29::sqr_addhi(r, x, y);
  else if (op == 7) F29::mul_addhi(r, x, y, y);
  else if (op == 9) { typename F29::fe c; F29::load(c, a + 2 * (size_t)i); F29::mul32(r, c); }
  else F29::mul(r, x, y);
  dbg_out29<F29>(out + 2 * (size_t)i, r);
}
template <class F>
__global__ void k_dbg_inv_lazy(const uint4* __restrict__ a, uint4* __restrict__ out, u32 n) {
  u32 i = blockIdx.x * blockDim.x + threadIdx.x;
  if (i >= n) return;
  typename F::fe x, r; F::load(x, a + 2 * (size_t)i);
  inv_via_lazy<F>(r, x);
  F::store(out + 2 * (size_t)i, r);
}
template <class G29>
__global__ void k_dbg_pointop29(int op, const char* __restrict__ acc_in, const char* __restrict__ q_in, char* __restrict__ out, u32 n) {
  typedef typename G29::F_ F29;
  u32 i = blockIdx.x * blockDim.x + threadIdx.x;
  if (i >= n) return;
  typename G29::pt acc;
  const char* ap = acc_in + (size_t)i * 128;
  dbg_in29<F29>(acc.x, ap); dbg_in29<F29>(acc.y, ap + 32); dbg_in29<F29>(acc.zz, ap + 64); dbg_in29<F29>(acc.zzz, ap + 96);
  if (G29::is_identity(acc)) G29::set_identity(acc);
  if (op == 0 || op == 2) {
    typename F29::fe xa, ya; F29::load(xa, q_in + (size_t)i * 64); F29::load(ya, q_in + (size_t)i * 64 + 32);
    if (!(F29::limbs_zero(xa) && F29::limbs_zero(ya))) {
      if (op == 0) { typename F29::fe x, y; F29::from_abi(x, xa); F29::from_abi(y, ya); G29::madd(acc, x, y); }
      else { G29::scale(acc); bool empty = G29::is_identity(acc); G29::madd_abi(acc, xa, ya, empty); G29::unscale(acc); }
    }
  } else {
    typename G29::pt q; const char* qp = q_in + (size_t)i * 128;
    dbg_in29<F29>(q.x, qp); dbg_in29<F29>(q.y, qp + 32); dbg_in29<F29>(q.zz, qp + 64); dbg_in29<F29>(q.zzz, qp + 96);
    if (G29::is_identity(q)) G29::set_identity(q);
    G29::add(acc, q);
  }
  char* op_ = out + (size_t)i * 128;
  if (G29::is_identity(acc)) { uint4 z = make_uint4(0, 0, 0, 0); for (int k = 0; k < 8; k++) reinterpret_cast<uint4*>(op_)[k] = z; return; }
  dbg_out29<F29>(op_, acc.x); dbg_out29<F29>(op_ + 32, acc.y); dbg_out29<F29>(op_ + 64, acc.zz); dbg_out29<F29>(op_ + 96, acc.zzz);
}

template <class F>
__global__ __launch_bounds__(256) void k_validate_points(const uint4* __restrict__ pts, u32 n, int bcoef , u32* __restrict__ err) {
  u32 j = blockIdx.x * 256 + threadIdx.x;
  if (j >= n) return;
  typedef typename F::fe fe;
  fe x, y; F::load(x, pts + (size_t)j * 4); F::load(y, pts + (size_t)j * 4 + 2);
  if (F::is_zero(x) && F::is_zero(y)) return;
  fe one, b, t, l, r; F::set_one(one); F::set_zero(b);
  int m = bcoef < 0 ? -bcoef : bcoef;
  for (int bit = 5; bit >= 0; bit--) { F::add(b, b, b); if ((m >> bit) & 1) F::add(b, b, one); }
  if (bcoef < 0) F::neg(b, b);
  F::sqr(l, y); F::sqr(t, x); F::mul(r, t, x); F::add(r, r, b);
  if (!F::eq(l, r)) atomicMin(err, j);
}

int validate_points(lemsm_ctx* ctx, int curve, const void* d_points, size_t n) {
  if (!ctx->opt_validate_points || n == 0) return LEMSM_OK;
  int rc = reserve(ctx, ctx->in_aux, 256); if (rc) return rc;
  u32 init = 0xffffffffu;
  HIPCHK(ctx, hipMemcpyAsync(ctx->in_aux.p, &init, 4, hipMemcpyHostToDevice, ctx->stream));
  HIPCHK(ctx, hipStreamSynchronize(ctx->stream));
  for (size_t s0 = 0; s0 < n; s0 += (size_t)1 << 30) {
    u32 cnt = (u32)std::min((size_t)1 << 30, n - s0);
    const uint4* p = (const uint4*)((const char*)d_points + s0 * 64);
    if (curve == LEMSM_BN254_G1) hipLaunchKernelGGL((k_validate_points<FqDev>), dim3((cnt + 255) / 256), dim3(256), 0, ctx->stream, p, cnt, 3, (u32*)ctx->in_aux.p);
    else hipLaunchKernelGGL((k_validate_points<FrDev>), dim3((cnt + 255) / 256), dim3(256), 0, ctx->stream, p, cnt, -17, (u32*)ctx->in_aux.p);
    u32 bad = 0xffffffffu;
    HIPCHK(ctx, hipMemcpyAsync(&bad, ctx->in_aux.p, 4, hipMemcpyDeviceToHost, ctx->stream));
    HIPCHK(ctx, hipStreamSynchronize(ctx->stream));
    if (bad != 0xffffffffu) { ctx->bad_index = s0 + bad; return fail(ctx, LEMSM_ERR_BAD_ARG, "point is not on the curve (option validate_points)"); }
  }
  return LEMSM_OK;
}

}

extern "C" {

const char* lemsm_strerror(int s) {
  switch (s) {
    case LEMSM_OK: return "ok";
    case LEMSM_ERR_LEN_MISMATCH: return "incompatible amount of coefficients";
    case LEMSM_ERR_SCALAR_OUT_OF_RANGE: return "scalar out of range";
    case LEMSM_ERR_BAD_BASE: return "base must be in 3..=255";
    case LEMSM_ERR_BAD_CURVE: return "unknown curve";
    case LEMSM_ERR_HIP: return "HIP runtime error";
    case LEMSM_ERR_BAD_ARG: return "bad argument";
    case LEMSM_ERR_NOMEM: return "out of device memory";
    case LEMSM_ERR_TOO_MANY_DIGITS: return "too many digits";
    case LEMSM_ERR_RCCL: return "RCCL error";
    case LEMSM_ERR_INDEX_OUT_OF_BOUNDS: return "index out of bounds";
    case LEMSM_ERR_ARITH_OVERFLOW: return "arithmetic overflow";
    case LEMSM_ERR_SUM_NOT_IDENTITY: return "points do not sum to the identity";
    case LEMSM_ERR_WOULD_NOT_TERMINATE: return "the reference would loop forever";
    case LEMSM_ERR_DIVISION_BY_ZERO: return "division by zero";
    default: return "unknown status";
  }
}

int lemsm_create(int device, lemsm_ctx** out) {
  if (!out) return LEMSM_ERR_BAD_ARG;
  *out = nullptr;
  int count = 0;
  if (hipGetDeviceCount(&count) != hipSuccess || count == 0 || device < 0 || device >= count) return LEMSM_ERR_HIP;
  hipDeviceProp_t prop;
  if (hipGetDeviceProperties(&prop, device) != hipSuccess) return LEMSM_ERR_HIP;
  if (strncmp(prop.gcnArchName, "gfx950", 6) != 0) return LEMSM_ERR_HIP;
  if (hipSetDevice(device) != hipSuccess) return LEMSM_ERR_HIP;
  lemsm_ctx* c = new lemsm_ctx();
  c->device = device;
  c->num_cus = prop.multiProcessorCount > 0 ? (u32)prop.multiProcessorCount : 256u;
  {
    int lo = 0, hi = 0;
    (void)hipDeviceGetStreamPriorityRange(&lo, &hi);
    if (hipStreamCreateWithPriority(&c->stream, hipStreamNonBlocking, lo) != hipSuccess ||
        hipStreamCreateWithPriority(&c->stream_sort, hipStreamNonBlocking, hi) != hipSuccess ||
        hipStreamCreateWithPriority(&c->stream_tail, hipStreamNonBlocking, hi) != hipSuccess) { delete c; return LEMSM_ERR_HIP; }
  }
  for (int i = 0; i < 5; i++) if (hipEventCreate(&c->ev[i]) != hipSuccess) { delete c; return LEMSM_ERR_HIP; }
  *out = c;
  return LEMSM_OK;
}

void lemsm_destroy(lemsm_ctx* ctx) {
  if (!ctx) return;
  (void)hipSetDevice(ctx->device);
  (void)hipStreamSynchronize(ctx->stream);
  if (ctx->stream_sort) { (void)hipStreamSynchronize(ctx->stream_sort); (void)hipStreamDestroy(ctx->stream_sort); }
  if (ctx->stream_tail) { (void)hipStreamSynchronize(ctx->stream_tail); (void)hipStreamDestroy(ctx->stream_tail); }
  for (hipEvent_t e : ctx->evpool) (void)hipEventDestroy(e);
  if (ctx->comm) { (void)Rccl::get().CommDestroy(ctx->comm); ctx->comm = nullptr; }
  if (ctx->peer) { lemsm_destroy(ctx->peer); ctx->peer = nullptr; }
  ctx->pool.reset();
  if (ctx->h_pin) (void)hipHostFree(ctx->h_pin);
  if (ctx->h_small) (void)hipHostFree(ctx->h_small);
  for (DevBuf* b : {&ctx->ws, &ctx->in_s, &ctx->in_p, &ctx->in_aux, &ctx->gather, &ctx->fail_buf, &ctx->dw_tab, &ctx->dw_arena, &ctx->dw_tmp}) if (b->p) (void)hipFree(b->p);
  for (auto& kv : ctx->pyr_cache) if (kv.second.buf.p) (void)hipFree(kv.second.buf.p);
  for (int i = 0; i < 5; i++) if (ctx->ev[i]) (void)hipEventDestroy(ctx->ev[i]);
  for (int i = 0; i < 2; i++) if (ctx->dw_ev[i]) (void)hipEventDestroy(ctx->dw_ev[i]);
  if (ctx->ev_batch_up) (void)hipEventDestroy(ctx->ev_batch_up);
  if (ctx->ev_call_done) (void)hipEventDestroy(ctx->ev_call_done);
  if (ctx->stream) (void)hipStreamDestroy(ctx->stream);
  delete ctx;
}

const char* lemsm_last_error(const lemsm_ctx* ctx) { return ctx ? ctx->last_error.c_str() : "null context"; }

int lemsm_set_option(lemsm_ctx* ctx, const char* name, long value) {
  if (!ctx || !name) return LEMSM_ERR_BAD_ARG;
  if (!strcmp(name, "window_bits")) { if (value != 0 && (value < 2 || value > 17)) return LEMSM_ERR_BAD_ARG; ctx->opt_window_bits = value; }
  else if (!strcmp(name, "chunk")) { if (value < 0 || value > 65536) return LEMSM_ERR_BAD_ARG; ctx->opt_chunk = value; }
  else if (!strcmp(name, "binsort")) { if (value < 0) return LEMSM_ERR_BAD_ARG; ctx->opt_binsort = value; }
  else if (!strcmp(name, "tile")) { if (value < 0 || (value && value < 256)) return LEMSM_ERR_BAD_ARG; ctx->opt_tile = value; }
  else if (!strcmp(name, "groups")) { if (value < 0 || value > 64) return LEMSM_ERR_BAD_ARG; ctx->opt_groups = value; }
  else if (!strcmp(name, "merge_slice")) { if (value != 0 && (value < 33 || value > 65536)) return LEMSM_ERR_BAD_ARG; ctx->opt_merge_slice = value; }
  else if (!strcmp(name, "dbg_repeat")) { ctx->opt_dbg_repeat = value; }
  else if (!strcmp(name, "pyr_first2")) { if (value < 0 || value > 1) return LEMSM_ERR_BAD_ARG; ctx->opt_pyr_first2 = value; }
  else if (!strcmp(name, "merge_wave_th")) { if (value < 0 || value > (1 << 24)) return LEMSM_ERR_BAD_ARG; ctx->opt_merge_wave_th = value; }
  else if (!strcmp(name, "abi_points")) { if (value < 0 || value > 2) return LEMSM_ERR_BAD_ARG; ctx->opt_abi_points = value; }
  else if (!strcmp(name, "stage2x")) { if (value < 0 || value > 4 || value == 3) return LEMSM_ERR_BAD_ARG; ctx->opt_stage2x = value; }
  else if (!strcmp(name, "xcd_windows")) { if (value < 0 || value > 1) return LEMSM_ERR_BAD_ARG; ctx->opt_xcd_windows = value; }
  else if (!strcmp(name, "ws_canary")) { if (value < 0 || value > 1) return LEMSM_ERR_BAD_ARG; ctx->opt_ws_canary = value; }
  else if (!strcmp(name, "dw_kb")) { if (value < 0 || value > 64) return LEMSM_ERR_BAD_ARG; ctx->opt_dw_kb = value; }
  else if (!strcmp(name, "dw_fuse")) { if (value != 0 && value != 2) return LEMSM_ERR_BAD_ARG; ctx->opt_dw_fuse = value; }
  else if (!strcmp(name, "dw_pw_lazy")) { if (value != 0 && value != 1) return LEMSM_ERR_BAD_ARG; ctx->opt_dw_pw_lazy = value; }
  else if (!strcmp(name, "scatter_lean")) { if (value < 0 || value > 1) return LEMSM_ERR_BAD_ARG; ctx->opt_scatter_lean = value; }
  else if (!strcmp(name, "pyr_quad")) { if (value != 0 && value != 2) return LEMSM_ERR_BAD_ARG; ctx->opt_pyr_quad = value; }
  else if (!strcmp(name, "slab_tail")) { if (value != 0 && value != 2) return LEMSM_ERR_BAD_ARG; ctx->opt_slab_tail = value; }
  else if (!strcmp(name, "dw_halves")) { if (value != 0 && value != 1) return LEMSM_ERR_BAD_ARG; ctx->opt_dw_halves = value; }
  else if (!strcmp(name, "dw_ntt_lazy")) { if (value != 0 && value != 1) return LEMSM_ERR_BAD_ARG; ctx->opt_dw_ntt_lazy = value; }
  else if (!strcmp(name, "dw_reuse")) { if (value != 0 && value != 2) return LEMSM_ERR_BAD_ARG; ctx->opt_dw_reuse = value; }
  else if (!strcmp(name, "dw_wrap")) { if (value != 0 && value != 2) return LEMSM_ERR_BAD_ARG; ctx->opt_dw_wrap = value; }
  else if (!strcmp(name, "ntt_tiled")) { if (value != 0 && value != 2) return LEMSM_ERR_BAD_ARG; ctx->opt_ntt_tiled = value; }
  else if (!strcmp(name, "pyr_fuse")) { if (value < 0 || value > 2) return LEMSM_ERR_BAD_ARG; ctx->opt_pyr_fuse = value; }
  else if (!strcmp(name, "validate_points")) { if (value < 0 || value > 1) return LEMSM_ERR_BAD_ARG; ctx->opt_validate_points = value; }
  else if (!strcmp(name, "entry_ring")) { if (value < 0 || value > 1) return LEMSM_ERR_BAD_ARG; ctx->opt_entry_ring = value; }
  else if (!strcmp(name, "slab_bits")) { if (value != 0 && (value < 12 || value > 24)) return LEMSM_ERR_BAD_ARG; ctx->opt_slab_bits = value; }
  else if (!strcmp(name, "host_slab_bits")) { if (value != 0 && (value < 12 || value > 24)) return LEMSM_ERR_BAD_ARG; ctx->opt_host_slab_bits = value; }
  else if (!strcmp(name, "accum_waves")) { if (value != 0 && (value < 2 || value > 4)) return LEMSM_ERR_BAD_ARG; ctx->opt_accum_waves = value; }
  else if (!strcmp(name, "host_threads")) { if (value < 0 || value > 64) return LEMSM_ERR_BAD_ARG; ctx->opt_host_threads = value; ctx->pool.reset(); }
  else if (!strcmp(name, "field")) { if (value != 0 && value != 1) return LEMSM_ERR_BAD_ARG; ctx->opt_field = value; }
  else return LEMSM_ERR_BAD_ARG;
  return LEMSM_OK;
}

size_t lemsm_last_bad_index(const lemsm_ctx* ctx) { return ctx ? ctx->bad_index : 0; }
size_t lemsm_last_truncated_count(const lemsm_ctx* ctx) { return ctx ? ctx->truncated : 0; }

int lemsm_last_timing(const lemsm_ctx* ctx, double out[3]) {
  if (!ctx || !out) return LEMSM_ERR_BAD_ARG;
  out[0] = ctx->t_total_ms; out[1] = ctx->t_accum_ms; out[2] = ctx->n_accum;
  return LEMSM_OK;
}

int lemsm_debug_last_merge_counts(const lemsm_ctx* ctx, uint64_t out[4]) {
  if (!ctx || !out) return LEMSM_ERR_BAD_ARG;
  for (int q = 0; q < 4; q++) out[q] = ctx->dbg_merge[q];
  if (getenv("LEMSM_DEBUG_STAMPS")) fprintf(stderr, "[lemsm] merge stamps (cycles): queues wave0: setup %u sum %u store %u n %u | final wave0: setup %u sum %u store %u n %u\n",
                                            ctx->dbg_stamps[0], ctx->dbg_stamps[1], ctx->dbg_stamps[2], ctx->dbg_stamps[3] & 0x7fffffffu, ctx->dbg_stamps[4], ctx->dbg_stamps[5], ctx->dbg_stamps[6], ctx->dbg_stamps[7]);
  return LEMSM_OK;
}

int lemsm_last_accum_clock_mhz(const lemsm_ctx* ctx, double* out) {
  if (!ctx || !out) return LEMSM_ERR_BAD_ARG;
  *out = ctx->accum_clock_mhz;
  return LEMSM_OK;
}

int lemsm_msm_plan(const lemsm_ctx* ctx, int curve, size_t n, uint32_t* num_windows, size_t* partial_bytes_per_window) {
  if (curve != LEMSM_BN254_G1 && curve != LEMSM_GRUMPKIN) return LEMSM_ERR_BAD_CURVE;
  MsmPlan mp = make_msm_plan(ctx, curve, n);
  if (num_windows) *num_windows = mp.W;
  if (partial_bytes_per_window) *partial_bytes_per_window = 128;
  return LEMSM_OK;
}

int lemsm_msm_partial_device(lemsm_ctx* ctx, int curve, const void* d_scalars, const void* d_points, size_t n,
                             uint32_t win_begin, uint32_t win_end, uint8_t* out_partials) {
  if (!ctx || (!out_partials && win_begin != win_end)) return LEMSM_ERR_BAD_ARG;
  int rc = check_curve(ctx, curve); if (rc) return rc;
  HIPCHK(ctx, hipSetDevice(ctx->device));
  std::vector<host::pt> out;
  rc = msm_partial_dispatch(ctx, curve, d_scalars, d_points, n, win_begin, win_end, out);
  if (rc) return rc;
  if (!out.empty()) memcpy(out_partials, out.data(), out.size() * sizeof(host::pt));
  return LEMSM_OK;
}

int lemsm_msm_combine(const lemsm_ctx* ctx, int curve, size_t n, const uint8_t* partials, uint64_t out[12]) {
  if (!partials || !out) return LEMSM_ERR_BAD_ARG;
  if (curve != LEMSM_BN254_G1 && curve != LEMSM_GRUMPKIN) return LEMSM_ERR_BAD_CURVE;
  MsmPlan mp = make_msm_plan(ctx, curve, n);
  std::vector<host::pt> recs((size_t)mp.W);
  memcpy(recs.data(), partials, recs.size() * sizeof(host::pt));
  if (curve == LEMSM_BN254_G1) msm_combine_t<host::FqParams64>(mp, recs.data(), out);
  else msm_combine_t<host::FrParams64>(mp, recs.data(), out);
  return LEMSM_OK;
}

int lemsm_msm_device(lemsm_ctx* ctx, int curve, const void* d_scalars, const void* d_points, size_t n, uint64_t out[12]) {
  if (!ctx || !out) return LEMSM_ERR_BAD_ARG;
  int rc = check_curve(ctx, curve); if (rc) return rc;
  if (n == 0) { memset(out, 0, 96); return LEMSM_OK; }
  HIPCHK(ctx, hipSetDevice(ctx->device));
  if (!(ctx->host_stage && ctx->host_stage->h_points)) { rc = validate_points(ctx, curve, d_points, n); if (rc) return rc; }
  MsmPlan mp = make_msm_plan(ctx, curve, n);
  std::vector<host::pt> sums;
  rc = msm_partial_dispatch(ctx, curve, d_scalars, d_points, n, 0, mp.W, sums);
  if (rc) return rc;
  const auto th0 = std::chrono::steady_clock::now();
  if (curve == LEMSM_BN254_G1) msm_combine_t<host::FqParams64>(mp, sums.data(), out);
  else msm_combine_t<host::FrParams64>(mp, sums.data(), out);
  ctx->host_us[3] = std::chrono::duration<double, std::micro>(std::chrono::steady_clock::now() - th0).count();
  if (getenv("LEMSM_DEBUG_STAMPS")) fprintf(stderr, "[lemsm] host tail (us): device wait %.1f, records + window sums %.1f, (unused) %.1f, Horner %.1f\n", ctx->host_us[0], ctx->host_us[1], ctx->host_us[2], ctx->host_us[3]);
  return LEMSM_OK;
}

struct lemsm_bases { lemsm_ctx* ctx; int device; int curve; size_t n; void* d_points; bool validated; };
static int msm_batch_entry(lemsm_ctx* ctx, int curve, const void* const* d_scalars, const uint8_t* const* h_scalars, const lemsm_bases* bases,
                           size_t batch, const void* d_points, size_t n, uint64_t* outs) {
  int rc = check_curve(ctx, curve); if (rc) return rc;
  if (batch == 0) return LEMSM_OK;
  if (n == 0) { memset(outs, 0, batch * 96); return LEMSM_OK; }
  for (size_t k = 0; k < batch; k++) if (h_scalars ? !h_scalars[k] : !d_scalars[k]) return LEMSM_ERR_BAD_ARG;
  HIPCHK(ctx, hipSetDevice(ctx->device));
  if (!(bases && bases->validated)) { rc = validate_points(ctx, curve, d_points, n); if (rc) return rc; }
  if (ctx->opt_field == 1 || ctx->opt_groups > 1 || batch == 1) {
    for (size_t k = 0; k < batch; k++) {
      rc = h_scalars ? lemsm_msm_with_bases(ctx, bases, h_scalars[k], n, outs + 12 * k) : lemsm_msm_device(ctx, curve, d_scalars[k], d_points, n, outs + 12 * k);
      if (rc) return rc;
    }
    return LEMSM_OK;
  }
  if (!ctx->peer) { rc = lemsm_create(ctx->device, &ctx->peer); if (rc) return fail(ctx, rc, "lemsm_msm_batch_device: second lane could not be created"); }
  {
    lemsm_ctx* p = ctx->peer;
    p->opt_window_bits = ctx->opt_window_bits; p->opt_chunk = ctx->opt_chunk; p->opt_tile = ctx->opt_tile; p->opt_field = ctx->opt_field;
    p->opt_accum_waves = ctx->opt_accum_waves; p->opt_groups = ctx->opt_groups; p->opt_slab_bits = ctx->opt_slab_bits; p->opt_abi_points = ctx->opt_abi_points;
    p->opt_stage2x = ctx->opt_stage2x; p->opt_xcd_windows = ctx->opt_xcd_windows; p->opt_entry_ring = ctx->opt_entry_ring; p->opt_pyr_fuse = ctx->opt_pyr_fuse;
    p->opt_ws_canary = ctx->opt_ws_canary; p->opt_binsort = ctx->opt_binsort; p->opt_merge_slice = ctx->opt_merge_slice; p->opt_merge_wave_th = ctx->opt_merge_wave_th;
    p->opt_pyr_first2 = ctx->opt_pyr_first2; p->opt_host_threads = ctx->opt_host_threads; p->plan_world = ctx->plan_world; p->opt_slab_tail = ctx->opt_slab_tail; p->opt_pyr_quad = ctx->opt_pyr_quad; p->opt_scatter_lean = ctx->opt_scatter_lean;
  }
  if (curve == LEMSM_BN254_G1) return msm_batch_t<host::FqParams64, GqLazy>(ctx, curve, d_scalars, d_points, n, batch, outs, h_scalars);
  return msm_batch_t<host::FrParams64, GrLazy>(ctx, curve, d_scalars, d_points, n, batch, outs, h_scalars);
}

int lemsm_msm_batch_device(lemsm_ctx* ctx, int curve, const void* const* d_scalars, size_t batch, const void* d_points, size_t n, uint64_t* outs) {
  if (!ctx || (batch && (!d_scalars || !outs))) return LEMSM_ERR_BAD_ARG;
  return msm_batch_entry(ctx, curve, d_scalars, nullptr, nullptr, batch, d_points, n, outs);
}

int lemsm_msm(lemsm_ctx* ctx, int curve, const uint8_t* scalars, const uint64_t* points, size_t n, uint64_t out[12]) {
  if (!ctx || !out || (n && (!scalars || !points))) return LEMSM_ERR_BAD_ARG;
  int rc = check_curve(ctx, curve); if (rc) return rc;
  if (n == 0) { memset(out, 0, 96); return LEMSM_OK; }
  HIPCHK(ctx, hipSetDevice(ctx->device));
  rc = reserve(ctx, ctx->in_s, n * 32); if (rc) return rc;
  rc = reserve(ctx, ctx->in_p, n * 64); if (rc) return rc;
  HostStage hs{scalars, points, (char*)ctx->in_s.p, (char*)ctx->in_p.p};
  if (ctx->opt_validate_points) {
    HIPCHK(ctx, hipMemcpy(ctx->in_p.p, points, n * 64, hipMemcpyHostToDevice));
    hs.h_points = nullptr;
  }
  ctx->host_stage = &hs;
  rc = lemsm_msm_device(ctx, curve, ctx->in_s.p, ctx->in_p.p, n, out);
  ctx->host_stage = nullptr;
  return rc;
}
int lemsm_msm_bn254_g1(lemsm_ctx* ctx, const uint8_t* s, const uint64_t* p, size_t n, uint64_t out[12]) { return lemsm_msm(ctx, LEMSM_BN254_G1, s, p, n, out); }
int lemsm_msm_grumpkin(lemsm_ctx* ctx, const uint8_t* s, const uint64_t* p, size_t n, uint64_t out[12]) { return lemsm_msm(ctx, LEMSM_GRUMPKIN, s, p, n, out); }

int lemsm_num_digits(int curve, uint8_t base, uint32_t* d) {
  if (curve != LEMSM_BN254_G1 && curve != LEMSM_GRUMPKIN) return LEMSM_ERR_BAD_CURVE;
  if (base < 2 || !d) return LEMSM_ERR_BAD_BASE;
  *d = logb_ceil8(bound_of(curve), base) + 1;
  return LEMSM_OK;
}

int lemsm_negbase_decompose_batch(lemsm_ctx* ctx, const uint8_t* scalars, size_t n, uint8_t base, uint32_t d, uint8_t* digits) {
  if (!ctx || (n && (!scalars || !digits))) return LEMSM_ERR_BAD_ARG;
  if (base < 2) return fail(ctx, LEMSM_ERR_BAD_BASE, "base must be >= 2");
  if (n == 0 || d == 0) return LEMSM_OK;
  if (n >= ((size_t)1 << 32)) return fail(ctx, LEMSM_ERR_BAD_ARG, "n too large");
  HIPCHK(ctx, hipSetDevice(ctx->device));
  int rc = stage(ctx, ctx->in_s, scalars, n * 32); if (rc) return rc;
  size_t dig_bytes = align_up((size_t)n * d, 256);
  rc = reserve(ctx, ctx->in_aux, dig_bytes + 256); if (rc) return rc;
  char* b = (char*)ctx->in_aux.p;
  u32 init[12] = {0, 0, 0, 0, 0, 0, 0, 0, 0xffffffffu, 0, 0xffffffffu, 0};
  HIPCHK(ctx, hipMemcpyAsync(b + dig_bytes, init, sizeof init, hipMemcpyHostToDevice, ctx->stream));
  HIPCHK(ctx, hipStreamSynchronize(ctx->stream));
  hipLaunchKernelGGL(k_negbase_digits, dim3((u32)((n + 255) / 256)), dim3(256), 0, ctx->stream, (const uint4*)ctx->in_s.p, (u32)n,
                     (u32)base, d, (const u32*)(b + dig_bytes), 0, (uint8_t*)b, (uint8_t*)nullptr, (u32*)(b + dig_bytes) + 8, 0u, d);
  HIPCHK(ctx, hipGetLastError());
  HIPCHK(ctx, hipMemcpyAsync(digits, b, (size_t)n * d, hipMemcpyDeviceToHost, ctx->stream));
  u32 errw[2] = {0, 0};
  HIPCHK(ctx, hipMemcpyAsync(errw, (u32*)(b + dig_bytes) + 8, 8, hipMemcpyDeviceToHost, ctx->stream));
  HIPCHK(ctx, hipStreamSynchronize(ctx->stream));
  ctx->truncated = errw[1];
  return LEMSM_OK;
}

int lemsm_prepare_scalar_witness_batch(lemsm_ctx* ctx, const uint8_t* scalars, const uint8_t* negative, size_t n, uint8_t base,
                                       uint32_t num_digits, uint32_t logtable, uint8_t* out_entries, size_t* bad_index) {
  if (!ctx || (n && (!scalars || !out_entries))) return LEMSM_ERR_BAD_ARG;
  if (base < 2) return fail(ctx, LEMSM_ERR_BAD_BASE, "base must be >= 2");
  if (logtable == 0) return fail(ctx, LEMSM_ERR_BAD_ARG, "logtable == 0: the reference divides by it (:82)");
  if (num_digits > 4096) return fail(ctx, LEMSM_ERR_BAD_ARG, "num_digits too large");
  if (n >= ((size_t)1 << 32)) return fail(ctx, LEMSM_ERR_BAD_ARG, "n too large");
  if (n == 0) return LEMSM_OK;
  const u32 d = num_digits, num_limbs = (num_digits + logtable - 1) / logtable, cols = num_limbs + 1;
  HIPCHK(ctx, hipSetDevice(ctx->device));
  std::vector<WitnessPow> pw(std::max<u32>(d, 1));
  {
    unsigned __int128 mag = 1; bool ovf = false;
    for (u32 e = 0; e < d; e++) {
      pw[e].ovf = ovf ? 1u : 0u; pw[e].pad = 0;
      __int128 v = (e & 1u) ? -(__int128)mag : (__int128)mag;
      pw[e].lo = (unsigned long long)(unsigned __int128)v; pw[e].hi = (long long)(v >> 64);
      if (!ovf) { unsigned __int128 nx = mag * base; if (nx / base != mag || nx >= ((unsigned __int128)1 << 127)) ovf = true; else mag = nx; }
    }
  }
  const size_t dig_bytes = align_up((size_t)n * std::max<u32>(d, 1), 256), flag_bytes = align_up(n, 256), pow_bytes = align_up(pw.size() * sizeof(WitnessPow), 256);
  const size_t out_bytes = (size_t)n * base * cols * 24;
  int rc = stage(ctx, ctx->in_s, scalars, n * 32); if (rc) return rc;
  rc = reserve(ctx, ctx->in_aux, dig_bytes + 2 * flag_bytes + pow_bytes + 512); if (rc) return rc;
  rc = reserve(ctx, ctx->ws, out_bytes + 256); if (rc) return rc;
  char* b = (char*)ctx->in_aux.p;
  uint8_t* d_digits = (uint8_t*)b; uint8_t* d_neg = (uint8_t*)(b + dig_bytes); uint8_t* d_trunc = d_neg + flag_bytes;
  WitnessPow* d_pow = (WitnessPow*)(b + dig_bytes + 2 * flag_bytes);
  u32* d_words = (u32*)(b + dig_bytes + 2 * flag_bytes + pow_bytes);
  u32 init[16] = {0, 0, 0, 0, 0, 0, 0, 0, 0xffffffffu, 0, 0xffffffffu, 0, 0xffffffffu, 0xffffffffu, 0, 0};
  HIPCHK(ctx, hipMemcpyAsync(d_words, init, sizeof init, hipMemcpyHostToDevice, ctx->stream));
  HIPCHK(ctx, hipMemcpyAsync(d_pow, pw.data(), pw.size() * sizeof(WitnessPow), hipMemcpyHostToDevice, ctx->stream));
  if (negative) HIPCHK(ctx, hipMemcpyAsync(d_neg, negative, n, hipMemcpyHostToDevice, ctx->stream));
  HIPCHK(ctx, hipStreamSynchronize(ctx->stream));
  dim3 grid((u32)((n + 255) / 256)), blk(256);
  hipLaunchKernelGGL(k_negbase_digits, grid, blk, 0, ctx->stream, (const uint4*)ctx->in_s.p, (u32)n, (u32)base, d, (const u32*)d_words, 0,
                     d_digits, (uint8_t*)nullptr, d_words + 8, 0u, 0u, negative ? (const uint8_t*)d_neg : (const uint8_t*)nullptr, d_trunc);
  hipLaunchKernelGGL(k_scalar_witness, grid, blk, 0, ctx->stream, (const uint4*)ctx->in_s.p, negative ? (const uint8_t*)d_neg : (const uint8_t*)nullptr,
                     (const uint8_t*)d_digits, (const uint8_t*)d_trunc, (u32)n, (u32)base, d, logtable, num_limbs, (const WitnessPow*)d_pow,
                     (char*)ctx->ws.p, (unsigned long long*)(d_words + 12));
  HIPCHK(ctx, hipGetLastError());
  unsigned long long failw = 0;
  HIPCHK(ctx, hipMemcpyAsync(&failw, d_words + 12, 8, hipMemcpyDeviceToHost, ctx->stream));
  HIPCHK(ctx, hipMemcpyAsync(out_entries, ctx->ws.p, out_bytes, hipMemcpyDeviceToHost, ctx->stream));
  HIPCHK(ctx, hipStreamSynchronize(ctx->stream));
  if (failw != ~0ull) {
    size_t j = (size_t)(failw >> 4); u32 code = (u32)(failw & 15u);
    if (bad_index) *bad_index = j;
    ctx->bad_index = j;
    if (code == 1) return fail(ctx, LEMSM_ERR_TOO_MANY_DIGITS, "negabase expansion longer than num_digits (assert at src/negbase_utils.rs:81)");
    if (code == 2) return fail(ctx, LEMSM_ERR_INDEX_OUT_OF_BOUNDS, "limb index i % logtable + 1 > num_limbs (index out of bounds at src/negbase_utils.rs:98-101)");
    return fail(ctx, LEMSM_ERR_ARITH_OVERFLOW, "i128 / u32 overflow in pow or += (src/negbase_utils.rs:97-101, a panic in the reference's debug build)");
  }
  return LEMSM_OK;
}

int lemsm_table_entries(lemsm_ctx* ctx, int curve, uint8_t base, uint64_t id_begin, size_t count, uint64_t* out) {
  if (!ctx || (count && !out)) return LEMSM_ERR_BAD_ARG;
  int rc = check_curve(ctx, curve); if (rc) return rc;
  if (count == 0) return LEMSM_OK;
  if (count >= ((size_t)1 << 31)) return fail(ctx, LEMSM_ERR_BAD_ARG, "count too large");
  HIPCHK(ctx, hipSetDevice(ctx->device));
  rc = reserve(ctx, ctx->ws, count * 32 + 256); if (rc) return rc;
  dim3 grid((u32)((count + 255) / 256)), blk(256);
  if (curve == LEMSM_BN254_G1) hipLaunchKernelGGL((k_table_entries<FqDev>), grid, blk, 0, ctx->stream, (u32)base, (unsigned long long)id_begin, (u32)count, (uint4*)ctx->ws.p);
  else hipLaunchKernelGGL((k_table_entries<FrDev>), grid, blk, 0, ctx->stream, (u32)base, (unsigned long long)id_begin, (u32)count, (uint4*)ctx->ws.p);
  HIPCHK(ctx, hipGetLastError());
  HIPCHK(ctx, hipMemcpyAsync(out, ctx->ws.p, count * 32, hipMemcpyDeviceToHost, ctx->stream));
  HIPCHK(ctx, hipStreamSynchronize(ctx->stream));
  return LEMSM_OK;
}

int lemsm_lhs_plan(int curve, uint8_t base, uint32_t* num_positions, size_t* partial_bytes) {
  if (curve != LEMSM_BN254_G1 && curve != LEMSM_GRUMPKIN) return LEMSM_ERR_BAD_CURVE;
  LhsPlan lp; int rc = make_lhs_plan(curve, base, lp); if (rc) return rc;
  if (num_positions) *num_positions = lp.d;
  if (partial_bytes) *partial_bytes = 128;
  return LEMSM_OK;
}

int lemsm_lhs_partial_device(lemsm_ctx* ctx, int curve, const void* d_scalars, const void* d_points, size_t n, uint8_t base,
                             uint32_t pos_begin, uint32_t pos_end, uint8_t* out_partials, size_t* bad_index) {
  if (!ctx || (!out_partials && pos_begin != pos_end)) return LEMSM_ERR_BAD_ARG;
  int rc = check_curve(ctx, curve); if (rc) return rc;
  LhsPlan lp; rc = make_lhs_plan(curve, base, lp); if (rc) return fail(ctx, rc, "base must be in 3..=255");
  HIPCHK(ctx, hipSetDevice(ctx->device));
  std::vector<host::pt> out;
  rc = lhs_partial_dispatch(ctx, curve, d_scalars, d_points, n, lp, pos_begin, pos_end, out, bad_index);
  if (rc) return rc;
  if (!out.empty()) memcpy(out_partials, out.data(), out.size() * sizeof(host::pt));
  return LEMSM_OK;
}

int lemsm_lhs_combine(int curve, uint8_t base, const uint8_t* partials, uint64_t out_carry[12], uint64_t* out_carries) {
  if (!partials || !out_carry) return LEMSM_ERR_BAD_ARG;
  if (curve != LEMSM_BN254_G1 && curve != LEMSM_GRUMPKIN) return LEMSM_ERR_BAD_CURVE;
  LhsPlan lp; int rc = make_lhs_plan(curve, base, lp); if (rc) return rc;
  std::vector<host::pt> recs((size_t)lp.d);
  memcpy(recs.data(), partials, recs.size() * sizeof(host::pt));
  if (curve == LEMSM_BN254_G1) lhs_combine_t<host::FqParams64>(lp, recs.data(), out_carry, out_carries);
  else lhs_combine_t<host::FrParams64>(lp, recs.data(), out_carry, out_carries);
  return LEMSM_OK;
}

int lemsm_lhs_msm_device(lemsm_ctx* ctx, int curve, const void* d_scalars, const void* d_points, size_t n, uint8_t base,
                         uint64_t out_carry[12], uint64_t* out_carries, size_t* bad_index) {
  if (!ctx || !out_carry) return LEMSM_ERR_BAD_ARG;
  int rc = check_curve(ctx, curve); if (rc) return rc;
  LhsPlan lp; rc = make_lhs_plan(curve, base, lp); if (rc) return fail(ctx, rc, "base must be in 3..=255");
  HIPCHK(ctx, hipSetDevice(ctx->device));
  rc = validate_points(ctx, curve, d_points, n); if (rc) return rc;
  std::vector<host::pt> recs;
  rc = lhs_partial_dispatch(ctx, curve, d_scalars, d_points, n, lp, 0, lp.d, recs, bad_index);
  if (rc) return rc;
  if (curve == LEMSM_BN254_G1) lhs_combine_t<host::FqParams64>(lp, recs.data(), out_carry, out_carries);
  else lhs_combine_t<host::FrParams64>(lp, recs.data(), out_carry, out_carries);
  return LEMSM_OK;
}

int lemsm_lhs_msm(lemsm_ctx* ctx, int curve, const uint8_t* scalars, const uint64_t* pts_jac, size_t n, uint8_t base,
                  uint64_t out_carry[12], uint64_t* out_carries, size_t* bad_index) {
  if (!ctx || !out_carry || (n && (!scalars || !pts_jac))) return LEMSM_ERR_BAD_ARG;
  int rc = check_curve(ctx, curve); if (rc) return rc;
  if (base < 3) return fail(ctx, LEMSM_ERR_BAD_BASE, "base must be in 3..=255");
  if (n >= ((size_t)1 << 32)) return fail(ctx, LEMSM_ERR_BAD_ARG, "n too large");
  HIPCHK(ctx, hipSetDevice(ctx->device));
  rc = stage(ctx, ctx->in_s, scalars, n * 32); if (rc) return rc;
  const int KB = 32;
  size_t nthreads = ((n + KB - 1) / KB + 255) / 256 * 256;
  size_t jac_bytes = align_up(n * 96, 256), scr_bytes = (size_t)KB * nthreads * 32;
  rc = reserve(ctx, ctx->ws, jac_bytes + scr_bytes + 256); if (rc) return rc;
  rc = reserve(ctx, ctx->in_p, n ? n * 64 : 16); if (rc) return rc;
  if (n) {
    HIPCHK(ctx, hipMemcpyAsync(ctx->ws.p, pts_jac, n * 96, hipMemcpyHostToDevice, ctx->stream));
    if (curve == LEMSM_BN254_G1)
      hipLaunchKernelGGL((k_jac_to_affine<FqDev, KB>), dim3((u32)(nthreads / 256)), dim3(256), 0, ctx->stream, (const uint4*)ctx->ws.p, (u32)n,
                         (uint4*)ctx->in_p.p, (char*)ctx->ws.p + jac_bytes);
    else
      hipLaunchKernelGGL((k_jac_to_affine<FrDev, KB>), dim3((u32)(nthreads / 256)), dim3(256), 0, ctx->stream, (const uint4*)ctx->ws.p, (u32)n,
                         (uint4*)ctx->in_p.p, (char*)ctx->ws.p + jac_bytes);
    HIPCHK(ctx, hipGetLastError());
    HIPCHK(ctx, hipStreamSynchronize(ctx->stream));
  }
  return lemsm_lhs_msm_device(ctx, curve, ctx->in_s.p, ctx->in_p.p, n, base, out_carry, out_carries, bad_index);
}
int lemsm_lhs_msm_grumpkin(lemsm_ctx* ctx, const uint8_t* s, const uint64_t* p, size_t n, uint8_t base, uint64_t oc[12], uint64_t* ocs, size_t* bad) {
  return lemsm_lhs_msm(ctx, LEMSM_GRUMPKIN, s, p, n, base, oc, ocs, bad);
}
int lemsm_lhs_msm_bn254_g1(lemsm_ctx* ctx, const uint8_t* s, const uint64_t* p, size_t n, uint8_t base, uint64_t oc[12], uint64_t* ocs, size_t* bad) {
  return lemsm_lhs_msm(ctx, LEMSM_BN254_G1, s, p, n, base, oc, ocs, bad);
}

int lemsm_comm_unique_id(uint8_t id[LEMSM_COMM_ID_BYTES]) {
  if (!id) return LEMSM_ERR_BAD_ARG;
  Rccl& R = Rccl::get();
  if (!R.ok()) return LEMSM_ERR_RCCL;
  static_assert(LEMSM_COMM_ID_BYTES == NCCL_UNIQUE_ID_BYTES, "unique id size");
  ncclUniqueId u;
  if (R.GetUniqueId(&u) != ncclSuccess) return LEMSM_ERR_RCCL;
  memcpy(id, u.internal, NCCL_UNIQUE_ID_BYTES);
  return LEMSM_OK;
}

int lemsm_comm_init(lemsm_ctx* ctx, const uint8_t id[LEMSM_COMM_ID_BYTES], int nranks, int rank) {
  if (!ctx || !id || nranks < 1 || rank < 0 || rank >= nranks) return LEMSM_ERR_BAD_ARG;
  Rccl& R = Rccl::get();
  if (!R.ok()) return fail(ctx, LEMSM_ERR_RCCL, "RCCL not loadable: " + R.error);
  if (ctx->comm) return fail(ctx, LEMSM_ERR_BAD_ARG, "context already has a communicator (lemsm_comm_destroy first)");
  HIPCHK(ctx, hipSetDevice(ctx->device));
  ncclUniqueId u; memcpy(u.internal, id, NCCL_UNIQUE_ID_BYTES);
  RCCLCHK(ctx, R.CommInitRank(&ctx->comm, nranks, u, rank));
  ctx->comm_size = nranks; ctx->comm_rank = rank;
  return LEMSM_OK;
}

int lemsm_comm_destroy(lemsm_ctx* ctx) {
  if (!ctx) return LEMSM_ERR_BAD_ARG;
  if (ctx->comm) {
    (void)hipSetDevice(ctx->device);
    (void)hipStreamSynchronize(ctx->stream);
    ncclResult_t r = Rccl::get().CommDestroy(ctx->comm);
    ctx->comm = nullptr; ctx->comm_size = 1; ctx->comm_rank = 0;
    if (r != ncclSuccess) return fail(ctx, LEMSM_ERR_RCCL, std::string("ncclCommDestroy: ") + Rccl::get().GetErrorString(r));
  }
  return LEMSM_OK;
}

int lemsm_comm_info(const lemsm_ctx* ctx, int* nranks, int* rank) {
  if (!ctx) return LEMSM_ERR_BAD_ARG;
  if (nranks) *nranks = ctx->comm ? ctx->comm_size : 0;
  if (rank) *rank = ctx->comm ? ctx->comm_rank : 0;
  return LEMSM_OK;
}

int lemsm_msm_sharded_device(lemsm_ctx* ctx, int curve, const void* d_scalars, const void* d_points, size_t n, uint64_t out[12]) {
  if (!ctx || !out) return LEMSM_ERR_BAD_ARG;
  int rc = check_curve(ctx, curve); if (rc) return rc;
  if (!ctx->comm) return fail(ctx, LEMSM_ERR_BAD_ARG, "no communicator: call lemsm_comm_init on every rank first");
  HIPCHK(ctx, hipSetDevice(ctx->device));
  Exchange ex{ctx->comm_size, ctx->comm_rank, false};
  return msm_sharded_dispatch(ctx, curve, d_scalars, d_points, n, ex, out);
}

int lemsm_lhs_msm_sharded_device(lemsm_ctx* ctx, int curve, const void* d_scalars, const void* d_points, size_t n, uint8_t base,
                                 uint64_t out_carry[12], uint64_t* out_carries, size_t* bad_index) {
  if (!ctx || !out_carry) return LEMSM_ERR_BAD_ARG;
  int rc = check_curve(ctx, curve); if (rc) return rc;
  LhsPlan lp; rc = make_lhs_plan(curve, base, lp); if (rc) return fail(ctx, rc, "base must be in 3..=255");
  if (!ctx->comm) return fail(ctx, LEMSM_ERR_BAD_ARG, "no communicator: call lemsm_comm_init on every rank first");
  HIPCHK(ctx, hipSetDevice(ctx->device));
  Exchange ex{ctx->comm_size, ctx->comm_rank, false};
  return lhs_sharded_dispatch(ctx, curve, d_scalars, d_points, n, lp, ex, out_carry, out_carries, bad_index);
}

int lemsm_debug_msm_sharded_sim(lemsm_ctx* ctx, int curve, const void* d_scalars, const void* d_points, size_t n, int world, uint64_t out[12]) {
  if (!ctx || !out || world < 1 || world > 64) return LEMSM_ERR_BAD_ARG;
  int rc = check_curve(ctx, curve); if (rc) return rc;
  HIPCHK(ctx, hipSetDevice(ctx->device));
  Exchange ex{world, 0, true};
  return msm_sharded_dispatch(ctx, curve, d_scalars, d_points, n, ex, out);
}
int lemsm_debug_lhs_sharded_sim(lemsm_ctx* ctx, int curve, const void* d_scalars, const void* d_points, size_t n, uint8_t base, int world,
                                uint64_t out_carry[12], uint64_t* out_carries, size_t* bad_index) {
  if (!ctx || !out_carry || world < 1 || world > 256) return LEMSM_ERR_BAD_ARG;
  int rc = check_curve(ctx, curve); if (rc) return rc;
  LhsPlan lp; rc = make_lhs_plan(curve, base, lp); if (rc) return fail(ctx, rc, "base must be in 3..=255");
  HIPCHK(ctx, hipSetDevice(ctx->device));
  Exchange ex{world, 0, true};
  return lhs_sharded_dispatch(ctx, curve, d_scalars, d_points, n, lp, ex, out_carry, out_carries, bad_index);
}


int lemsm_bases_upload(lemsm_ctx* ctx, int curve, const uint64_t* points_affine, size_t n, lemsm_bases** out) {
  if (!ctx || !out || (n && !points_affine)) return LEMSM_ERR_BAD_ARG;
  *out = nullptr;
  int rc = check_curve(ctx, curve); if (rc) return rc;
  HIPCHK(ctx, hipSetDevice(ctx->device));
  void* d = nullptr;
  hipError_t e = hipMalloc(&d, n ? n * 64 : 64);
  if (e != hipSuccess) return fail(ctx, LEMSM_ERR_NOMEM, hipGetErrorString(e));
  if (n) { e = hipMemcpy(d, points_affine, n * 64, hipMemcpyHostToDevice); if (e != hipSuccess) { (void)hipFree(d); return fail(ctx, LEMSM_ERR_HIP, hipGetErrorString(e)); } }
  if (ctx->opt_validate_points) { rc = validate_points(ctx, curve, d, n); if (rc) { (void)hipFree(d); return rc; } }
// ... 384 lines not shown
```

halo2_liam_eagen_msm_amd/csrc/plan.h:

```cpp
#pragma once
#include <stdint.h>

namespace lemsm {

static const uint32_t MAX_BINS = 8192;
static const uint32_t MAX_LB = 7;
static const uint32_t MAX_SLAB_LOG = 24;

struct GroupPlan {
  uint32_t n;
  uint32_t c;
  uint32_t nb;
  uint32_t nbw;
  uint32_t BW;
  uint32_t w0, w1;
  uint32_t W;
  uint32_t NB;
  uint32_t LB;
  uint32_t nbins;
  uint32_t spb;
  uint32_t nblk1;
  uint32_t T2;
  uint32_t max_tiles;
  uint32_t bin_cap;
  uint32_t L1;
  uint32_t nthr1;
  uint32_t d;
  uint32_t dstride;
  uint32_t nstride;
};

struct PyrTask {
  uint32_t src_off, src_wstride;
  uint32_t dst_off, dst_wstride;
  uint32_t stride, phase, count, src_valid;
  uint32_t src_scaled, pad_[3];
};
struct CopyTask { uint32_t src_off, src_wstride, dst_off, dst_wstride, src_valid_idx, src_idx; };

struct MqLayout { uint32_t offS, offM, offL, offF, capS, capM, capL, capF, capP, slice, wave_th; };

}
```

Measured before the change: 886.4 million.

## Fuse digit extraction, bin counting and scatter into one kernel with fixed bin regions

```diff
diff --git a/halo2_liam_eagen_msm_amd/csrc/kernels.cuh b/halo2_liam_eagen_msm_amd/csrc/kernels.cuh
--- a/halo2_liam_eagen_msm_amd/csrc/kernels.cuh
+++ b/halo2_liam_eagen_msm_amd/csrc/kernels.cuh
@@ -23,8 +23,10 @@
 __global__ __launch_bounds__(BS) void k_pip_digits(const uint4* __restrict__ scalars, KAdd kadd, GroupPlan pl,
                                                     uint16_t* __restrict__ dig16, unsigned long long* __restrict__ signbm,
                                                     u32* __restrict__ block_counts,
-                                                    u32* __restrict__ bin_total, u32* __restrict__ err) {
+                                                    u32* __restrict__ bin_total, u32* __restrict__ err,
+                                                    const u32* __restrict__ gate = nullptr) {
   __shared__ u32 hist[MAX_BINS];
+  if (gate && !*gate) return;
   const u32 tid = threadIdx.x, r = blockIdx.x;
   for (u32 i = tid; i < pl.nbins; i += BS) hist[i] = 0;
   __syncthreads();
@@ -210,8 +212,9 @@
 
 __global__ __launch_bounds__(1024) void k_binscan(GroupPlan pl, const u32* __restrict__ bin_total,
                                                   u32* __restrict__ bin_start, u32* __restrict__ tile_prefix,
-                                                  u32* __restrict__ meta) {
+                                                  u32* __restrict__ meta, const u32* __restrict__ gate = nullptr) {
   __shared__ u32 wsum[16];
+  if (gate && !*gate) return;
   const u32 t = threadIdx.x;
   constexpr int PB = MAX_BINS / 1024;
   u32 cnt[PB], tl[PB], s = 0, st = 0;
@@ -241,7 +244,8 @@
           bool LEAN = false >
 __global__ __launch_bounds__(BS) void k_scatter1(Dec dec, GroupPlan pl, const u32* __restrict__ block_counts,
                                                  const u32* __restrict__ bin_start,
-                                                 u32* __restrict__ entries, u32 xcd_windows ) {
+                                                 u32* __restrict__ entries, u32 xcd_windows ,
+                                                 const u32* __restrict__ gate = nullptr) {
   static_assert(BS == 256 || BS == 1024, "block size");
   static_assert(STG <= 16384, "jl field is 14 bits");
   static_assert(!LEAN || BS == 256, "the lean form is the 256-thread one");
@@ -249,6 +253,7 @@
   __shared__ __align__(8) u32 lcur[BW_MAX];
   __shared__ u32 wsum[16];
   __shared__ u32 stage[STG];
+  if (gate && !*gate) return;
   const u32 tid = threadIdx.x;
   u32 wl, r;
   if (xcd_windows) {
@@ -375,9 +380,146 @@
   }
 }
 
+__host__ __device__ inline u32 region_base(const GroupPlan& pl, u32 i) {
+  return i < pl.top_start ? i * pl.bin_cap : pl.top_start * pl.bin_cap + (i - pl.top_start < pl.top_bins ? i - pl.top_start : pl.top_bins) * pl.rtop;
+}
+__host__ __device__ inline u32 region_cap(const GroupPlan& pl, u32 i) {
+  return i < pl.top_start ? pl.bin_cap : (i - pl.top_start < pl.top_bins ? pl.rtop : 0u);
+}
+template <int MODE >
+__device__ __forceinline__ void pip_digit(const u32 (&s)[8], int w, u32 W, u32& bucket, u32& sign) {
+  const bool top = !((u32)w + 1 < W);
+  if (MODE == 2) {
+    const u32 raw = extract_bits(s, 17u * w, 17u);
+    sign = (!top && raw < 65536u) ? 1u : 0u;
+    bucket = top ? raw : (sign ? 65536u - raw : raw - 65536u);
+  } else {
+    const u32 raw = (w & 1) ? (s[w >> 1] >> 16) : (s[w >> 1] & 0xffffu);
+    sign = (!top && raw < 32768u) ? 1u : 0u;
+    bucket = top ? raw : (sign ? 32768u - raw : raw - 32768u);
+  }
+}
+
+template <int MODE , int BS, int PER, u32 NBMAX >
+__global__ __launch_bounds__(BS) void k_pip_fused(const uint4* __restrict__ scalars, KAdd kadd, GroupPlan pl,
+                                                  u32* __restrict__ bin_total, u32* __restrict__ entries,
+                                                  u32* __restrict__ err, u32* __restrict__ ovf) {
+  constexpr u32 S = (u32)BS * PER;
+  constexpr int NW = MODE == 2 ? 15 : 16;
+  static_assert(S <= 16384, "jl field is 14 bits");
+  __shared__ u32 cur[NBMAX];
+  __shared__ u32 dl[NBMAX];
+  __shared__ u32 stage[2 * S];
+  __shared__ u32 tot[16];
+  __shared__ u32 bad;
+  const u32 tid = threadIdx.x;
+  const u32 j0 = blockIdx.x * S, j1 = min(j0 + S, pl.n);
+  u32 s[PER][8];
+#pragma unroll
+  for (int k = 0; k < PER; k++) {
+    const u32 j = j0 + tid + (u32)BS * k;
+    uint4 a = make_uint4(0, 0, 0, 0), b = a;
+    if (j < j1) { a = scalars[2 * (size_t)j]; b = scalars[2 * (size_t)j + 1]; }
+    s[k][0] = a.x; s[k][1] = a.y; s[k][2] = a.z; s[k][3] = a.w; s[k][4] = b.x; s[k][5] = b.y; s[k][6] = b.z; s[k][7] = b.w;
+  }
+  for (u32 i = tid; i < pl.nbins; i += BS) cur[i] = 0;
+  if (tid == 0) bad = 0;
+#pragma unroll
+  for (int k = 0; k < PER; k++) {
+    u32 bw = 0;
+#pragma unroll
+    for (int i = 0; i < 8; i++) { u32 dmy = __builtin_subc(s[k][i], kadd.order[i], bw, &bw); (void)dmy; }
+    if (!bw) {
+      atomicAdd(&err[0], 1u); atomicMax(&err[1], ~(j0 + tid + (u32)BS * k));
+#pragma unroll
+      for (int i = 0; i < 8; i++) s[k][i] = 0;
+    }
+    u32 cy = 0;
+#pragma unroll
+    for (int i = 0; i < 8; i++) s[k][i] = __builtin_addc(s[k][i], kadd.k[i], cy, &cy);
+  }
+  __syncthreads();
+#pragma unroll
+  for (int w = 0; w < NW; w++) {
+    if ((u32)w < pl.w0 || (u32)w >= pl.w1) continue;
+    u32* h = cur + ((u32)w - pl.w0) * pl.BW;
+#pragma unroll
+    for (int k = 0; k < PER; k++) {
+      u32 bucket, sign;
+      pip_digit<MODE>(s[k], w, pl.W, bucket, sign);
+      if (bucket) atomicAdd(&h[(bucket - 1u) >> pl.LB], 1u);
+    }
+  }
+  __syncthreads();
+  {
+    const u32 lane = tid & 63u, gw = pl.w1 - pl.w0, PB = pl.BW >> 6;
+    bool over = false;
+    for (u32 wl = tid >> 6; wl < gw; wl += BS / 64) {
+      const u32 i0 = wl * pl.BW + lane * PB;
+      u32 c[8], g[8], sum = 0;
+#pragma unroll
+      for (int p = 0; p < 8; p++) {
+        c[p] = (u32)p < PB ? cur[i0 + p] : 0u;
+        g[p] = (u32)p < PB ? atomicAdd(&bin_total[i0 + p], c[p]) : 0u;
+        sum += c[p];
+      }
+      u32 x = sum;
+#pragma unroll
+      for (int o = 1; o < 64; o <<= 1) { u32 y = __shfl_up(x, o); if (lane >= (u32)o) x += y; }
+      if (lane == 63) tot[wl] = x;
+      u32 off = x - sum;
+#pragma unroll
+      for (int p = 0; p < 8; p++) {
+        if ((u32)p < PB) {
+          over |= c[p] && g[p] + c[p] > region_cap(pl, i0 + p);
+          cur[i0 + p] = off;
+          dl[i0 + p] = region_base(pl, i0 + p) + g[p] - off;
+          off += c[p];
+        }
+      }
+    }
+    if (over) bad = 1u;
+  }
+  __syncthreads();
+  if (bad) {
+    if (tid == 0) *ovf = 1u;
+    return;
+  }
+  const u32 lmask = (1u << pl.LB) - 1u;
+#pragma unroll
+  for (int w = 0; w < NW; w++) {
+    if ((u32)w < pl.w0 || (u32)w >= pl.w1) continue;
+    const u32 wl = (u32)w - pl.w0;
+    u32* buf = stage + (wl & 1u) * S;
+    u32* cw = cur + wl * pl.BW;
+#pragma unroll
+    for (int k = 0; k < PER; k++) {
+      u32 bucket, sign;
+      pip_digit<MODE>(s[k], w, pl.W, bucket, sign);
+      if (bucket) {
+        const u32 kk = bucket - 1u, b = kk >> pl.LB;
+        buf[atomicAdd(&cw[b], 1u)] = (tid + (u32)BS * k) | ((kk & lmask) << 14) | (sign << 21) | (b << 22);
+      }
+    }
+    __syncthreads();
+    const u32 total = tot[wl];
+    const u32* dw = dl + wl * pl.BW;
+#pragma unroll
+    for (int k = 0; k < PER; k++) {
+      const u32 q = tid + (u32)BS * k;
+      if (q < total) {
+        const u32 v = buf[q];
+        entries[dw[v >> 22] + q] = (j0 + (v & 0x3fffu)) | (((v >> 14) & 127u) << 24) | (((v >> 21) & 1u) << 31);
+      }
+    }
+  }
+}
+
 __global__ __launch_bounds__(256) void k_tilemap(GroupPlan pl, const u32* __restrict__ bin_start,
                                                  const u32* __restrict__ tile_prefix, const u32* __restrict__ meta,
-                                                 uint4* __restrict__ tile_info) {
+                                                 uint4* __restrict__ tile_info, const u32* __restrict__ gate = nullptr, u32 run_if_set = 1,
+                                                 u32 fixed = 0 ) {
+  if (gate && (*gate != 0) != (run_if_set != 0)) return;
   u32 t = blockIdx.x * 256 + threadIdx.x;
   if (t >= pl.max_tiles) return;
   if (t >= meta[META_TILES]) { tile_info[t] = make_uint4(0, 0, 0, 0); return; }
@@ -386,8 +528,9 @@
     u32 mid = (lo + hi) >> 1;
     if (tile_prefix[mid] <= t) lo = mid; else hi = mid;
   }
-  u32 off = bin_start[lo] + (t - tile_prefix[lo]) * pl.T2;
-  u32 end = min(off + pl.T2, bin_start[lo + 1]);
+  const u32 b0 = bin_start[lo], base = fixed ? region_base(pl, lo) : b0;
+  u32 off = base + (t - tile_prefix[lo]) * pl.T2;
+  u32 end = min(off + pl.T2, base + (bin_start[lo + 1] - b0));
   tile_info[t] = make_uint4(lo, off, end, 1u);
 }
 __device__ __forceinline__ bool locate_tile(const uint4* __restrict__ tile_info, u32 t, u32& bin, u32& off, u32& end) {
@@ -397,8 +540,10 @@
 }
 
 __global__ __launch_bounds__(256) void k_count2(GroupPlan pl, const u32* __restrict__ entries,
-                                                const uint4* __restrict__ tile_info, u32* __restrict__ bucket_count) {
+                                                const uint4* __restrict__ tile_info, u32* __restrict__ bucket_count,
+                                                const u32* __restrict__ gate = nullptr, u32 run_if_set = 1) {
   __shared__ u32 hist[1u << MAX_LB];
+  if (gate && (*gate != 0) != (run_if_set != 0)) return;
   const u32 tid = threadIdx.x;
   for (u32 t = blockIdx.x; t < pl.max_tiles; t += gridDim.x) {
     u32 bin, off, end;
@@ -422,9 +567,10 @@
 
 __global__ __launch_bounds__(256) void k_bucketscan(GroupPlan pl, const u32* __restrict__ bin_start,
                                                     const u32* __restrict__ bucket_count,
-                                                    u32* __restrict__ bucket_start) {
+                                                    u32* __restrict__ bucket_start, const u32* __restrict__ gate = nullptr, u32 run_if_set = 1) {
   __shared__ u32 ex[256];
   __shared__ u32 wsum[4];
+  if (gate && (*gate != 0) != (run_if_set != 0)) return;
   const u32 tid = threadIdx.x;
   const u32 key = blockIdx.x * 256 + tid;
   const u32 nkeys = pl.nbins << pl.LB;
@@ -444,12 +590,14 @@
 
 __global__ __launch_bounds__(256) void k_scatter2(GroupPlan pl, const u32* __restrict__ entries,
                                                   const uint4* __restrict__ tile_info, const u32* __restrict__ bucket_start,
-                                                  u32* __restrict__ bucket_cursor, u32* __restrict__ sorted) {
+                                                  u32* __restrict__ bucket_cursor, u32* __restrict__ sorted,
+                                                  const u32* __restrict__ gate = nullptr, u32 run_if_set = 1) {
   __shared__ u32 hist[256];
   __shared__ u32 lstart[257];
   __shared__ u32 delta[256];
   __shared__ u32 wsum[4];
   __shared__ u32 stage[STAGE2];
+  if (gate && (*gate != 0) != (run_if_set != 0)) return;
   const u32 tid = threadIdx.x;
   for (u32 t = blockIdx.x; t < pl.max_tiles; t += gridDim.x) {
     u32 bin, off, end;
@@ -495,21 +643,25 @@
 static const u32 BIN_CAP_SMALL = 8192;
 template <u32 CAP>
 __global__ __launch_bounds__(1024) void k_binsort(GroupPlan pl, const u32* __restrict__ entries, const u32* __restrict__ bin_start,
-                                                  u32* __restrict__ sorted, u32* __restrict__ bucket_start) {
+                                                  u32* __restrict__ sorted, u32* __restrict__ bucket_start,
+                                                  u32 fixed ,
+                                                  const u32* __restrict__ gate = nullptr, u32 run_if_set = 1) {
   __shared__ u32 stage[CAP];
   __shared__ u32 hist[256];
   __shared__ u32 lstart[256];
   __shared__ u32 wsum[4];
+  if (gate && (*gate != 0) != (run_if_set != 0)) return;
   const u32 tid = threadIdx.x, bin = blockIdx.x;
   const u32 off = bin_start[bin], end = bin_start[bin + 1], cnt = end - off;
   if (cnt > pl.bin_cap) return;
+  const u32* __restrict__ src = entries + (fixed ? region_base(pl, bin) : off);
   const u32 nl = 1u << pl.LB, lmask = nl - 1u;
   if (tid < 256) hist[tid] = 0;
   __syncthreads();
   constexpr int PER = CAP / 1024;
   u32 e[PER], rk[PER];
 #pragma unroll
-  for (int k = 0; k < PER; k++) { u32 i = off + tid + 1024u * k; e[k] = i < end ? entries[i] : 0u; }
+  for (int k = 0; k < PER; k++) { u32 i = off + tid + 1024u * k; e[k] = i < end ? src[i - off] : 0u; }
 #pragma unroll
   for (int k = 0; k < PER; k++) {
     u32 i = off + tid + 1024u * k;
diff --git a/halo2_liam_eagen_msm_amd/csrc/lemsm.hip b/halo2_liam_eagen_msm_amd/csrc/lemsm.hip
--- a/halo2_liam_eagen_msm_amd/csrc/lemsm.hip
+++ b/halo2_liam_eagen_msm_amd/csrc/lemsm.hip
@@ -108,7 +108,7 @@
   std::unique_ptr<lemsm::host::Pool> pool;
   std::string last_error;
   long opt_host_threads = 0;
-  long opt_window_bits = 0, opt_chunk = 0, opt_tile = 0, opt_field = 0, opt_accum_waves = 0, opt_groups = 0, opt_host_slab_bits = 0, opt_slab_bits = 0, opt_abi_points = 0, opt_stage2x = 0, opt_xcd_windows = 0, opt_entry_ring = 0, opt_validate_points = 0, opt_pyr_fuse = 0, opt_ntt_tiled = 0, opt_ws_canary = 0, opt_binsort = 0, opt_dw_wrap = 0, opt_dw_fuse = 0, opt_dw_kb = 0, opt_merge_slice = 0, opt_merge_wave_th = 0, opt_dbg_repeat = 0, opt_pyr_first2 = 0, opt_dw_reuse = 0, opt_dw_pw_lazy = 0, opt_dw_halves = 0, opt_dw_ntt_lazy = 0, opt_slab_tail = 0, opt_pyr_quad = 0, opt_scatter_lean = 0;
+  long opt_window_bits = 0, opt_chunk = 0, opt_tile = 0, opt_field = 0, opt_accum_waves = 0, opt_groups = 0, opt_host_slab_bits = 0, opt_slab_bits = 0, opt_abi_points = 0, opt_stage2x = 0, opt_xcd_windows = 0, opt_entry_ring = 0, opt_validate_points = 0, opt_pyr_fuse = 0, opt_ntt_tiled = 0, opt_ws_canary = 0, opt_binsort = 0, opt_dw_wrap = 0, opt_dw_fuse = 0, opt_dw_kb = 0, opt_merge_slice = 0, opt_merge_wave_th = 0, opt_dbg_repeat = 0, opt_pyr_first2 = 0, opt_dw_reuse = 0, opt_dw_pw_lazy = 0, opt_dw_halves = 0, opt_dw_ntt_lazy = 0, opt_slab_tail = 0, opt_pyr_quad = 0, opt_scatter_lean = 0, opt_sort_fused = 1;
   u32 plan_slab_n = 0;
   bool plan_ring = false;
   const struct HostStage* host_stage = nullptr;
@@ -294,12 +294,18 @@
   w.zero_bytes_counters = o_arena - z0;
   size_t o_bin_start = take((MAX_BINS + 1) * 4), o_tile_prefix = take((MAX_BINS + 1) * 4), o_meta = take(64);
   size_t o_bstart = take(((size_t)NBpad + 1) * 4);
-  size_t o_blockc = take((size_t)pl.nblk1 * pl.nbins * 8);
-  size_t o_dig = take(pl.c ? (size_t)pl.dstride * (pl.w1 - pl.w0) * 2 + 64 : 16);
+  const size_t b_blockc = (size_t)pl.nblk1 * pl.nbins * 8;
+  const size_t b_dig = pl.c ? (size_t)pl.dstride * (pl.w1 - pl.w0) * 2 + 64 : 16;
+  const size_t b_sbm = pl.c == 17 ? (size_t)(pl.w1 - pl.w0) * ((pl.n + 63) / 64) * 8 + 16 : 16;
+  size_t Mmax = (size_t)pl.n * (pl.w1 - pl.w0);
+  const size_t b_sorted = Mmax * 4 + 4 * (size_t)pl.L1 + 512;
+  const bool alias = pl.fused && !guard;
   size_t o_tinfo = take((size_t)pl.max_tiles * 16 + 16);
-  size_t o_sbm = take(pl.c == 17 ? (size_t)(pl.w1 - pl.w0) * ((pl.n + 63) / 64) * 8 + 16 : 16);
-  size_t Mmax = (size_t)pl.n * (pl.w1 - pl.w0);
-  size_t o_entries = take(Mmax * 4 + 4 * (size_t)pl.L1 + 512), o_sorted = take(Mmax * 4 + 4 * (size_t)pl.L1 + 512);
+  size_t o_blockc = 0, o_dig = 0, o_sbm = 0;
+  if (!alias) { o_blockc = take(b_blockc); o_dig = take(b_dig); o_sbm = take(b_sbm); }
+  size_t o_entries = take(std::max(Mmax, pl.fused ? (size_t)region_base(pl, pl.nbins) : (size_t)0) * 4 + 4 * (size_t)pl.L1 + 512);
+  size_t o_sorted = take(alias ? std::max(b_sorted, align_up(b_blockc, 256) + align_up(b_dig, 256) + b_sbm) : b_sorted);
+  if (alias) { o_blockc = o_sorted; o_dig = o_blockc + align_up(b_blockc, 256); o_sbm = o_dig + align_up(b_dig, 256); }
   w.mq = mq;
   size_t o_rk = take((size_t)pl.nthr1 * 4 + 16), o_rp = take(2 * (size_t)pl.nthr1 * ptb + 256);
   size_t o_mqi = take(((size_t)mq.offF + mq.capF) * 16), o_mqp = take((size_t)mq.capP * ptb + 256);
@@ -367,6 +373,27 @@
   g.L1 = L1;
   g.nthr1 = (u32)((Mmax + L1 - 1) / L1);
   if (g.nthr1 == 0) g.nthr1 = 1;
+  g.fused = (ctx->opt_sort_fused != 0 && d == 0 && LB > 0 && g.bin_cap && ((c == 17 && W == 15) || (c == 16 && W == 16)) &&
+             g.BW % 64 == 0 && g.BW <= 512 && g.nbins <= MAX_BINS && w1 - w0 <= 16) ? 1u : 0u;
+  g.top_start = g.nbins; g.top_bins = 0; g.rtop = 0;
+  if (g.fused && w1 == W) {
+    u32 top = nb;
+    for (int curve : {LEMSM_BN254_G1, LEMSM_GRUMPKIN}) {
+      const u32* order = order_of(curve);
+      u32 sum[9]; u64 cy = 0;
+      for (int i = 0; i < 8; i++) {
+        u32 k = 0;
+        for (u32 w = 0; w + 1 < W; w++) { u32 bit = w * c + c - 1; if ((bit >> 5) == (u32)i) k |= 1u << (bit & 31); }
+        cy += (u64)order[i] + k - (i == 0 ? 1u : 0u); sum[i] = (u32)cy; cy >>= 32;
+      }
+      u64 v = 0;
+      for (int bit = 255; bit >= (int)(c * (W - 1)); bit--) v = (v << 1) | ((sum[bit >> 5] >> (bit & 31)) & 1u);
+      top = std::min<u32>(top, (u32)std::max<u64>(1, v));
+    }
+    g.top_start = (W - 1 - w0) * g.BW;
+    g.top_bins = (top + (1u << LB) - 1) >> LB;
+    g.rtop = std::max<u32>(g.bin_cap, (u32)(((u64)n << LB) / std::max(1u, top / 2) * 9 / 8 + 1024));
+  }
   return g;
 }
 
@@ -380,25 +407,36 @@
 struct PipProvider {
   const uint4* scalars; KAdd kadd;
   typedef PipDec Dec;
+  void fused(hipStream_t st, const GroupPlan& pl, u32* bin_total, u32* entries, u32* err, u32* ovf) const {
+    const bool big = pl.n >= (1u << 23) || pl.nbins > 4096;
+    const u32 S = big ? 8192u : 2048u, grid = (pl.n + S - 1) / S;
+    if (pl.c == 17) {
+      if (big) hipLaunchKernelGGL((k_pip_fused<2, 1024, 8, MAX_BINS>), dim3(grid), dim3(1024), 0, st, scalars, kadd, pl, bin_total, entries, err, ovf);
+      else hipLaunchKernelGGL((k_pip_fused<2, 256, 8, 4096>), dim3(grid), dim3(256), 0, st, scalars, kadd, pl, bin_total, entries, err, ovf);
+    } else {
+      if (big) hipLaunchKernelGGL((k_pip_fused<1, 1024, 8, MAX_BINS>), dim3(grid), dim3(1024), 0, st, scalars, kadd, pl, bin_total, entries, err, ovf);
+      else hipLaunchKernelGGL((k_pip_fused<1, 256, 8, 4096>), dim3(grid), dim3(256), 0, st, scalars, kadd, pl, bin_total, entries, err, ovf);
+    }
+  }
   int prepare(lemsm_ctx*, hipStream_t st, const GroupPlan& pl, uint16_t* dig16, unsigned long long* signbm, u32* block_counts,
-              u32* bin_total, u32* err, Dec& dec) const {
+              u32* bin_total, u32* err, Dec& dec, const u32* gate = nullptr) const {
     dec.dig16 = dig16; dec.signbm = nullptr;
     if (pl.c == 17) {
       dec.signbm = signbm;
       if (pl.nblk1 < 2048)
-        hipLaunchKernelGGL((k_pip_digits<2, 1024>), dim3(pl.nblk1), dim3(1024), 0, st, scalars, kadd, pl, dig16, signbm, block_counts, bin_total, err);
+        hipLaunchKernelGGL((k_pip_digits<2, 1024>), dim3(pl.nblk1), dim3(1024), 0, st, scalars, kadd, pl, dig16, signbm, block_counts, bin_total, err, gate);
       else
-        hipLaunchKernelGGL((k_pip_digits<2>), dim3(pl.nblk1), dim3(256), 0, st, scalars, kadd, pl, dig16, signbm, block_counts, bin_total, err);
+        hipLaunchKernelGGL((k_pip_digits<2>), dim3(pl.nblk1), dim3(256), 0, st, scalars, kadd, pl, dig16, signbm, block_counts, bin_total, err, gate);
     } else if (pl.c == 16 && pl.W == 16) {
       if (pl.nblk1 < 1024)
-        hipLaunchKernelGGL((k_pip_digits<1, 1024>), dim3(pl.nblk1), dim3(1024), 0, st, scalars, kadd, pl, dig16, signbm, block_counts, bin_total, err);
+        hipLaunchKernelGGL((k_pip_digits<1, 1024>), dim3(pl.nblk1), dim3(1024), 0, st, scalars, kadd, pl, dig16, signbm, block_counts, bin_total, err, gate);
       else
-        hipLaunchKernelGGL((k_pip_digits<1>), dim3(pl.nblk1), dim3(256), 0, st, scalars, kadd, pl, dig16, signbm, block_counts, bin_total, err);
+        hipLaunchKernelGGL((k_pip_digits<1>), dim3(pl.nblk1), dim3(256), 0, st, scalars, kadd, pl, dig16, signbm, block_counts, bin_total, err, gate);
     } else {
       if (pl.nblk1 < 1024)
-        hipLaunchKernelGGL((k_pip_digits<0, 1024>), dim3(pl.nblk1), dim3(1024), 0, st, scalars, kadd, pl, dig16, signbm, block_counts, bin_total, err);
+        hipLaunchKernelGGL((k_pip_digits<0, 1024>), dim3(pl.nblk1), dim3(1024), 0, st, scalars, kadd, pl, dig16, signbm, block_counts, bin_total, err, gate);
       else
-        hipLaunchKernelGGL((k_pip_digits<0>), dim3(pl.nblk1), dim3(256), 0, st, scalars, kadd, pl, dig16, signbm, block_counts, bin_total, err);
+        hipLaunchKernelGGL((k_pip_digits<0>), dim3(pl.nblk1), dim3(256), 0, st, scalars, kadd, pl, dig16, signbm, block_counts, bin_total, err, gate);
     }
     return LEMSM_OK;
   }
@@ -406,7 +444,9 @@
 struct NegProvider {
   const uint8_t* digitsT;
   typedef NegDec Dec;
-  int prepare(lemsm_ctx*, hipStream_t st, const GroupPlan& pl, uint16_t*, unsigned long long*, u32* block_counts, u32* bin_total, u32*, Dec& dec) const {
+  void fused(hipStream_t, const GroupPlan&, u32*, u32*, u32*, u32*) const {}
+  int prepare(lemsm_ctx*, hipStream_t st, const GroupPlan& pl, uint16_t*, unsigned long long*, u32* block_counts, u32* bin_total, u32*, Dec& dec,
+              const u32* = nullptr) const {
     dec.digitsT = digitsT;
     hipLaunchKernelGGL((k_count1<NegDec>), dim3(pl.w1 - pl.w0, pl.nblk1), dim3(256), 0, st, dec, pl, block_counts, bin_total);
     return LEMSM_OK;
@@ -467,29 +507,42 @@
   for (size_t g : w.guards) HIPCHK(ctx, hipMemsetAsync(ws_base + g, 0xA5, WS_GUARD, st));
 
   typename Prov::Dec dec;
-  { int rcp = prov.prepare(ctx, st, pl, w.dig16, w.signbm, w.block_counts, w.bin_total, w.err, dec); if (rcp) return rcp; }
-  hipLaunchKernelGGL(k_binscan, dim3(1), dim3(1024), 0, st, pl, w.bin_total, w.bin_start, w.tile_prefix, w.meta);
+  u32* const ovf = pl.fused ? w.err + 2 : nullptr;
+  if (pl.fused) {
+    prov.fused(st, pl, w.bin_total, w.entries, w.err, ovf);
+    hipLaunchKernelGGL(k_binscan, dim3(1), dim3(1024), 0, st, pl, w.bin_total, w.bin_start, w.tile_prefix, w.meta, nullptr);
+    if (pl.bin_cap <= BIN_CAP_SMALL) hipLaunchKernelGGL((k_binsort<BIN_CAP_SMALL>), dim3(pl.nbins), dim3(1024), 0, st, pl, w.entries, w.bin_start, w.sorted, w.bucket_start, 1u, ovf, 0u);
+    else hipLaunchKernelGGL((k_binsort<BIN_CAP>), dim3(pl.nbins), dim3(1024), 0, st, pl, w.entries, w.bin_start, w.sorted, w.bucket_start, 1u, ovf, 0u);
+    hipLaunchKernelGGL(k_tilemap, dim3((pl.max_tiles + 255) / 256), dim3(256), 0, st, pl, w.bin_start, w.tile_prefix, w.meta, w.tile_info, ovf, 0u, 1u);
+    const u32 g2 = std::min(pl.max_tiles, 768u);
+    hipLaunchKernelGGL(k_count2, dim3(g2), dim3(256), 0, st, pl, w.entries, w.tile_info, w.bucket_count, ovf, 0u);
+    hipLaunchKernelGGL(k_bucketscan, dim3(((pl.nbins << pl.LB) + 255) / 256), dim3(256), 0, st, pl, w.bin_start, w.bucket_count, w.bucket_start, ovf, 0u);
+    hipLaunchKernelGGL(k_scatter2, dim3(g2), dim3(256), 0, st, pl, w.entries, w.tile_info, w.bucket_start, w.bucket_cursor, w.sorted, ovf, 0u);
+  }
+  u32* const totals = pl.fused ? w.bin_cursor : w.bin_total;
+  { int rcp = prov.prepare(ctx, st, pl, w.dig16, w.signbm, w.block_counts, totals, pl.fused ? w.err + 4 : w.err, dec, ovf); if (rcp) return rcp; }
+  hipLaunchKernelGGL(k_binscan, dim3(1), dim3(1024), 0, st, pl, totals, w.bin_start, w.tile_prefix, w.meta, ovf);
   const u32 xw = (gw >= 8 && ctx->opt_xcd_windows != 1) ? 1u : 0u;
   dim3 g1 = xw ? dim3(8u * ((gw + 7) / 8) * pl.nblk1) : dim3(gw, pl.nblk1);
   if (pl.spb > 2 * STAGE)
-    hipLaunchKernelGGL((k_scatter1<typename Prov::Dec, 4 * STAGE, 1024>), g1, dim3(1024), 0, st, dec, pl, w.block_counts, w.bin_start, w.entries, xw);
+    hipLaunchKernelGGL((k_scatter1<typename Prov::Dec, 4 * STAGE, 1024>), g1, dim3(1024), 0, st, dec, pl, w.block_counts, w.bin_start, w.entries, xw, ovf);
   else if (pl.spb > STAGE)
-    hipLaunchKernelGGL((k_scatter1<typename Prov::Dec, 2 * STAGE>), g1, dim3(256), 0, st, dec, pl, w.block_counts, w.bin_start, w.entries, xw);
+    hipLaunchKernelGGL((k_scatter1<typename Prov::Dec, 2 * STAGE>), g1, dim3(256), 0, st, dec, pl, w.block_counts, w.bin_start, w.entries, xw, ovf);
   else if (Prov::Dec::VEC && (pl.BW & 1u) == 0 && ctx->opt_scatter_lean == 1)
-    hipLaunchKernelGGL((k_scatter1<typename Prov::Dec, STAGE, 256, true>), g1, dim3(256), 0, st, dec, pl, w.block_counts, w.bin_start, w.entries, xw);
+    hipLaunchKernelGGL((k_scatter1<typename Prov::Dec, STAGE, 256, true>), g1, dim3(256), 0, st, dec, pl, w.block_counts, w.bin_start, w.entries, xw, ovf);
   else
-    hipLaunchKernelGGL((k_scatter1<typename Prov::Dec, STAGE>), g1, dim3(256), 0, st, dec, pl, w.block_counts, w.bin_start, w.entries, xw);
+    hipLaunchKernelGGL((k_scatter1<typename Prov::Dec, STAGE>), g1, dim3(256), 0, st, dec, pl, w.block_counts, w.bin_start, w.entries, xw, ovf);
   const u32* d_sorted = w.entries;
   const u32* d_bstart = w.bin_start;
   if (pl.LB > 0) {
-    if (pl.bin_cap && pl.bin_cap <= BIN_CAP_SMALL) hipLaunchKernelGGL((k_binsort<BIN_CAP_SMALL>), dim3(pl.nbins), dim3(1024), 0, st, pl, w.entries, w.bin_start, w.sorted, w.bucket_start);
-    else if (pl.bin_cap) hipLaunchKernelGGL((k_binsort<BIN_CAP>), dim3(pl.nbins), dim3(1024), 0, st, pl, w.entries, w.bin_start, w.sorted, w.bucket_start);
-    hipLaunchKernelGGL(k_tilemap, dim3((pl.max_tiles + 255) / 256), dim3(256), 0, st, pl, w.bin_start, w.tile_prefix, w.meta, w.tile_info);
+    if (pl.bin_cap && pl.bin_cap <= BIN_CAP_SMALL) hipLaunchKernelGGL((k_binsort<BIN_CAP_SMALL>), dim3(pl.nbins), dim3(1024), 0, st, pl, w.entries, w.bin_start, w.sorted, w.bucket_start, 0u, ovf, 1u);
+    else if (pl.bin_cap) hipLaunchKernelGGL((k_binsort<BIN_CAP>), dim3(pl.nbins), dim3(1024), 0, st, pl, w.entries, w.bin_start, w.sorted, w.bucket_start, 0u, ovf, 1u);
+    hipLaunchKernelGGL(k_tilemap, dim3((pl.max_tiles + 255) / 256), dim3(256), 0, st, pl, w.bin_start, w.tile_prefix, w.meta, w.tile_info, ovf, 1u, 0u);
     const u32 g2 = pl.bin_cap ? std::min(pl.max_tiles, 768u) : pl.max_tiles;
-    hipLaunchKernelGGL(k_count2, dim3(g2), dim3(256), 0, st, pl, w.entries, w.tile_info, w.bucket_count);
-    hipLaunchKernelGGL(k_bucketscan, dim3(((pl.nbins << pl.LB) + 255) / 256), dim3(256), 0, st, pl, w.bin_start, w.bucket_count, w.bucket_start);
+    hipLaunchKernelGGL(k_count2, dim3(g2), dim3(256), 0, st, pl, w.entries, w.tile_info, w.bucket_count, ovf, 1u);
+    hipLaunchKernelGGL(k_bucketscan, dim3(((pl.nbins << pl.LB) + 255) / 256), dim3(256), 0, st, pl, w.bin_start, w.bucket_count, w.bucket_start, ovf, 1u);
     hipLaunchKernelGGL(k_scatter2, dim3(g2), dim3(256), 0, st, pl, w.entries, w.tile_info,
-                       w.bucket_start, w.bucket_cursor, w.sorted);
+                       w.bucket_start, w.bucket_cursor, w.sorted, ovf, 1u);
     d_sorted = w.sorted; d_bstart = w.bucket_start;
   }
 
@@ -1476,6 +1529,7 @@
   else if (!strcmp(name, "dw_fuse")) { if (value != 0 && value != 2) return LEMSM_ERR_BAD_ARG; ctx->opt_dw_fuse = value; }
   else if (!strcmp(name, "dw_pw_lazy")) { if (value != 0 && value != 1) return LEMSM_ERR_BAD_ARG; ctx->opt_dw_pw_lazy = value; }
   else if (!strcmp(name, "scatter_lean")) { if (value < 0 || value > 1) return LEMSM_ERR_BAD_ARG; ctx->opt_scatter_lean = value; }
+  else if (!strcmp(name, "sort_fused")) { if (value < 0 || value > 1) return LEMSM_ERR_BAD_ARG; ctx->opt_sort_fused = value; }
   else if (!strcmp(name, "pyr_quad")) { if (value != 0 && value != 2) return LEMSM_ERR_BAD_ARG; ctx->opt_pyr_quad = value; }
   else if (!strcmp(name, "slab_tail")) { if (value != 0 && value != 2) return LEMSM_ERR_BAD_ARG; ctx->opt_slab_tail = value; }
   else if (!strcmp(name, "dw_halves")) { if (value != 0 && value != 1) return LEMSM_ERR_BAD_ARG; ctx->opt_dw_halves = value; }
@@ -1590,7 +1644,7 @@
     p->opt_accum_waves = ctx->opt_accum_waves; p->opt_groups = ctx->opt_groups; p->opt_slab_bits = ctx->opt_slab_bits; p->opt_abi_points = ctx->opt_abi_points;
     p->opt_stage2x = ctx->opt_stage2x; p->opt_xcd_windows = ctx->opt_xcd_windows; p->opt_entry_ring = ctx->opt_entry_ring; p->opt_pyr_fuse = ctx->opt_pyr_fuse;
     p->opt_ws_canary = ctx->opt_ws_canary; p->opt_binsort = ctx->opt_binsort; p->opt_merge_slice = ctx->opt_merge_slice; p->opt_merge_wave_th = ctx->opt_merge_wave_th;
-    p->opt_pyr_first2 = ctx->opt_pyr_first2; p->opt_host_threads = ctx->opt_host_threads; p->plan_world = ctx->plan_world; p->opt_slab_tail = ctx->opt_slab_tail; p->opt_pyr_quad = ctx->opt_pyr_quad; p->opt_scatter_lean = ctx->opt_scatter_lean;
+    p->opt_pyr_first2 = ctx->opt_pyr_first2; p->opt_host_threads = ctx->opt_host_threads; p->plan_world = ctx->plan_world; p->opt_slab_tail = ctx->opt_slab_tail; p->opt_pyr_quad = ctx->opt_pyr_quad; p->opt_scatter_lean = ctx->opt_scatter_lean; p->opt_sort_fused = ctx->opt_sort_fused;
   }
   if (curve == LEMSM_BN254_G1) return msm_batch_t<host::FqParams64, GqLazy>(ctx, curve, d_scalars, d_points, n, batch, outs, h_scalars);
   return msm_batch_t<host::FrParams64, GrLazy>(ctx, curve, d_scalars, d_points, n, batch, outs, h_scalars);
diff --git a/halo2_liam_eagen_msm_amd/csrc/plan.h b/halo2_liam_eagen_msm_amd/csrc/plan.h
--- a/halo2_liam_eagen_msm_amd/csrc/plan.h
+++ b/halo2_liam_eagen_msm_amd/csrc/plan.h
@@ -28,6 +28,8 @@
   uint32_t d;
   uint32_t dstride;
   uint32_t nstride;
+  uint32_t fused;
+  uint32_t top_start, top_bins, rtop;
 };
 
 struct PyrTask {
```

Result: faster. 900.2 million, median of 6 (+1.6%).
